# katotetsuro/chainer-maskrcnn

Hardware: AMD Instinct MI355X
Metric: images/sec (1024^2 COCO, bs=2/GPU) at 1/2/4/8 MI355X; ROIAlign bwd HBM GB/s (higher is better)
Workload: dtype f32

## Files before the change

__graft_entry__.py:

```python
import os
import subprocess
import sys

ROOT = os.path.dirname(os.path.abspath(__file__))
PKG = os.path.join(ROOT, 'chainer-maskrcnn_amd')
for _p in (ROOT, PKG):
    if _p not in sys.path:
        sys.path.insert(0, _p)


def build():
    csrc = os.path.join(PKG, 'csrc')
    subprocess.check_call(['make', '-C', csrc, '-j8'])
    oc = os.path.join(ROOT, 'oracle', 'c')
    if os.path.exists(os.path.join(oc, 'Makefile')):
        subprocess.check_call(['make', '-C', oc])
    from chainer_maskrcnn import _hip
    _hip._lib = None
    assert _hip.lib().mrcnn_abi_version() == _hip.ABI_VERSION


def smoke():
    import numpy as np
    import torch
    from chainer_maskrcnn.functions.roi_align_2d_yx import _roi_align_2d_yx
    from oracle import roi_align as ora
    if not torch.cuda.is_available():
        raise RuntimeError('smoke() needs a HIP device')
    rs = np.random.RandomState(0)
    x = rs.standard_normal((1, 256, 25, 34)).astype(np.float32)
    yx = np.array([[0, 10, 20, 300, 400], [0, 0, 0, 399, 543], [0, 100.5, 50.25, 130, 90]], np.float32)
    gy = rs.standard_normal((3, 256, 7, 7)).astype(np.float32)
    xt = torch.from_numpy(x).cuda().contiguous(memory_format=torch.channels_last).requires_grad_(True)
    y = _roi_align_2d_yx(xt, torch.from_numpy(yx).cuda(), 7, 7, 1. / 16)
    y.backward(torch.from_numpy(gy).cuda())
    xy = yx[:, [0, 2, 1, 4, 3]]
    np.testing.assert_array_equal(y.detach().cpu().numpy(), ora.roi_align_fwd(x, xy, 7, 7, 1. / 16, 2))
    np.testing.assert_allclose(xt.grad.cpu().numpy(), ora.roi_align_bwd(gy, xy, x.shape, 1. / 16, 2),
                               rtol=1e-5, atol=1e-4)
    print('smoke ok: roi_align fwd bit-exact, bwd within 1e-5 of the oracle')
    _smoke_train_step()


def _smoke_train_step():
    import numpy as np
    import torch
    from chainer_maskrcnn.model.maskrcnn import MaskRCNN
    from chainer_maskrcnn.model.fpn_maskrcnn_train_chain import FPNMaskRCNNTrainChain, calc_mask_loss
    from chainer_maskrcnn.optimizers import MomentumSGD, WeightDecay
    from chainer_maskrcnn.utils.synthetic import make_batch
    from oracle.model import OracleStep, D
    dev = 'cuda:0'
    stages = (1, 1, 1, 1)
    m = MaskRCNN(n_fg_class=80, device=dev, seed=3, _test_shrink=dict(stages=stages, width_div=2))
    chain = FPNMaskRCNNTrainChain(m, mask_loss_fun=calc_mask_loss, gemm_arithmetic='bf16x6_behind_backbone')
    opt = MomentumSGD(lr=1e-3, momentum=0.9).setup(chain)
    opt.add_hook(WeightDecay(0.0005))
    b = make_batch(3, 2, 128, 160, G=3)
    b['bboxes'][:, :, 2:] = np.minimum(b['bboxes'][:, :, 2:], [128, 160])
    bt = {k: torch.from_numpy(v).to(dev) for k, v in b.items()}
    params = {n: m.ps.p(n).detach().cpu().to(D) for n in m.ps.names()}
    opt.update(chain, bt['imgs'], bt['bboxes'], bt['labels'], bt['masks'], 1.0)
    obs = {k: float(v) for k, v in chain.observation.items()}
    t = {k: v.cpu().numpy() for k, v in chain.targets.items() if torch.is_tensor(v)}
    t['gt_rpn_loc'], t['gt_rpn_label'] = (x.cpu().numpy() for x in chain.rpn_targets)
    t['mask_rois_xy5'], t['mask_levels'], t['mask_label'] = (x.cpu().numpy() for x in chain.mask_inputs)
    img4 = torch.cat([torch.from_numpy(b['imgs']).permute(0, 2, 3, 1), torch.zeros((2, 128, 160, 1))], -1).to(D)
    with torch.no_grad():
        out = OracleStep(params, stages, m.head.n_class, m.head.LOC0).losses(img4, t)
    for k in ('rpn_loc_loss', 'rpn_cls_loss', 'roi_loc_loss', 'roi_cls_loss', 'mask_loss'):
        want = float(out[k])
        assert abs(obs[k] - want) <= 1e-4 * max(abs(want), 1e-3), (k, obs[k], want)
    assert torch.isfinite(m.ps.params).all()
    print('smoke ok: training step losses within 1e-4 of the oracle: %s' % {k: round(v, 5) for k, v in obs.items()})


if __name__ == '__main__':
    build()
    if len(sys.argv) > 1 and sys.argv[1] == 'smoke':
        smoke()
```

chainer-maskrcnn_amd/chainer_maskrcnn/_hip/nn.py:

```python
import torch

from chainer_maskrcnn import _hip
from chainer_maskrcnn._hip import lib, check, ptr, stream_ptr

_ws_cache = {}

PROFILE = None
LOGICAL = None


class _prof(object):
    def __init__(self, kind, n_out_pix, KH, KW, cin, cout, geom=None):
        self.on = PROFILE is not None
        if self.on:
            pass_ = {'fwd': 0, 'bwd_data': 1, 'bwd_filter': 2}[kind]
            executed = lib().mrcnn_conv2d_executed_macs(*geom, pass_) if geom is not None else n_out_pix * KH * KW * cin * cout
            if LOGICAL is not None:
                cin, cout = LOGICAL
            self.rec = [kind, n_out_pix * KH * KW * cin * cout, torch.cuda.Event(enable_timing=True),
                        torch.cuda.Event(enable_timing=True), (n_out_pix, KH, cin, cout), executed, geom,
                        winograd_pass_tiles(),
                        split_operands()]

    def __enter__(self):
# ... 29 lines not shown
        buf = torch.empty(max(int(nbytes), 1 << 20), dtype=torch.uint8, device=device)
        _ws_cache[key] = buf
    return buf


def winograd_pass_tiles():
    import ctypes
    t = (ctypes.c_int * 3)()
    check(lib().mrcnn_conv2d_get_winograd_pass_tiles(t))
    return (t[0], t[1], t[2])


def split_operands():
    import ctypes
    t = (ctypes.c_int * 3)()
    check(lib().mrcnn_conv2d_get_split_operands(t))
    return (t[0], t[1], t[2])


def set_winograd_pass_tiles(fwd, bwd_data, bwd_filter):
    check(lib().mrcnn_conv2d_set_winograd_pass_tiles(int(fwd), int(bwd_data), int(bwd_filter)))


def conv_out(n, k, s, p):
    return (n + 2 * p - k) // s + 1


CONV_PLAN_FIELDS = ('path', 'bm', 'bn', 'ksplit', 'tail_ks', 'wino_m', 'smallc', 'arithmetic', 'plane_gemm')
CONV_PATHS = ('direct', 'split_k', 'tail_split', 'winograd')


def conv_plan(pass_, x_shape, w_shape, stride, pad):
    import ctypes
    N, H, W, Cin = x_shape
    Cout, KH, KW, _ = w_shape
    out = (ctypes.c_int * len(CONV_PLAN_FIELDS))()
    check(lib().mrcnn_conv2d_plan_query(int(pass_), N, H, W, Cin, Cout, KH, KW, stride, pad, out, len(CONV_PLAN_FIELDS)))
    return dict(zip(CONV_PLAN_FIELDS, out))


def conv2d_fwd_raw(x, w, b, stride, pad, relu, keep_v=False):
    _hip.require_cuda(x, w)
    N, H, W, Cin = x.shape
    Cout, KH, KW, Cin2 = w.shape
    assert Cin == Cin2, (x.shape, w.shape)
    assert x.is_contiguous() and w.is_contiguous()
    y = torch.empty((N, conv_out(H, KH, stride, pad), conv_out(W, KW, stride, pad), Cout),
                    dtype=torch.float32, device=x.device)
    nb = lib().mrcnn_conv2d_workspace_bytes(N, H, W, Cin, Cout, KH, KW, stride, pad)
    ws = workspace(nb, x.device) if nb else None
    v = None
    if keep_v:
        vb = lib().mrcnn_conv2d_winograd_v_bytes(N, H, W, Cin, Cout, KH, KW, stride, pad)
        if vb:
            v = torch.empty((vb // 4,), dtype=torch.float32, device=x.device)
    with _prof('fwd', N * y.shape[1] * y.shape[2], KH, KW, Cin, Cout, (N, H, W, Cin, Cout, KH, KW, stride, pad)):
        check(lib().mrcnn_conv2d_fwd_f32(ptr(x), ptr(w), ptr(b), ptr(y), N, H, W, Cin, Cout, KH, KW,
                                         stride, pad, int(relu), ptr(v), ptr(ws), ws.numel() if ws is not None else 0, stream_ptr()))
    return (y, v) if keep_v else y


def conv2d_fwd_bnstats_raw(x, w, stride, pad, keep_v=False):
    N, H, W, Cin = x.shape
    Cout, KH, KW, _ = w.shape
    rows = lib().mrcnn_conv2d_bnstats_rows(N, H, W, Cin, Cout, KH, KW, stride, pad)
    if rows == 0:
        return None
    assert x.is_contiguous() and w.is_contiguous()
    y = torch.empty((N, conv_out(H, KH, stride, pad), conv_out(W, KW, stride, pad), Cout), dtype=torch.float32, device=x.device)
    part = torch.empty((rows, 2, Cout), dtype=torch.float32, device=x.device)
    nb = lib().mrcnn_conv2d_workspace_bytes(N, H, W, Cin, Cout, KH, KW, stride, pad)
    ws = workspace(nb, x.device) if nb else None
    v = None
    if keep_v:
        vb = lib().mrcnn_conv2d_winograd_v_bytes(N, H, W, Cin, Cout, KH, KW, stride, pad)
        if vb:
            v = torch.empty((vb // 4,), dtype=torch.float32, device=x.device)
    with _prof('fwd', N * y.shape[1] * y.shape[2], KH, KW, Cin, Cout, (N, H, W, Cin, Cout, KH, KW, stride, pad)):
        check(lib().mrcnn_conv2d_fwd_bnstats_f32(ptr(x), ptr(w), ptr(y), N, H, W, Cin, Cout, KH, KW, stride, pad, ptr(part), ptr(v),
                                                 ptr(ws), ws.numel() if ws is not None else 0, stream_ptr()))
    return y, v, part


def winograd_w_bytes(x_shape, w_shape, stride, pad):
    N, H, W, Cin = x_shape
    Cout, KH, KW, _ = w_shape
    return lib().mrcnn_conv2d_winograd_w_bytes(N, H, W, Cin, Cout, KH, KW, stride, pad)


def conv2d_bwd_data_raw(gy, w, x_shape, stride, pad, out=None, relu_x=None, emit_w=False, gb=None, gb_accumulate=False):
    N, H, W, Cin = x_shape
    Cout, KH, KW, _ = w.shape
    assert gy.is_contiguous()
    acc = out is not None
    gx = out if acc else torch.empty(x_shape, dtype=torch.float32, device=gy.device)
    nb = lib().mrcnn_conv2d_workspace_bytes(N, H, W, Cin, Cout, KH, KW, stride, pad)
    ws = workspace(nb, gy.device) if nb else None
    wt = None
    if emit_w:
        wb = lib().mrcnn_conv2d_winograd_w_bytes(N, H, W, Cin, Cout, KH, KW, stride, pad)
        assert wb > 0, 'emit_w: the layer does not take the Winograd path'
        wt = torch.empty((wb // 4,), dtype=torch.float32, device=gy.device)
    with _prof('bwd_data', N * gy.shape[1] * gy.shape[2], KH, KW, Cin, Cout, (N, H, W, Cin, Cout, KH, KW, stride, pad)):
        check(lib().mrcnn_conv2d_bwd_data_f32(ptr(gy), ptr(w), ptr(gx), ptr(relu_x), N, H, W, Cin, Cout, KH, KW,
                                              stride, pad, int(acc), ptr(wt), ptr(gb) if emit_w else None, int(gb_accumulate),
                                              ptr(ws), ws.numel() if ws is not None else 0, stream_ptr()))
    return (gx, wt) if emit_w else gx


def conv2d_bwd_filter_raw(x, gy, w_shape, stride, pad, want_bias, gw=None, gb=None, accumulate=None, wino_v=None,
                          wino_w=None):
    N, H, W, Cin = x.shape
    Cout, KH, KW, _ = w_shape
    assert gy.is_contiguous() and x.is_contiguous()
    acc = (gw is not None) if accumulate is None else bool(accumulate)
    if gw is None:
        gw = torch.empty(w_shape, dtype=torch.float32, device=x.device)
        gb = torch.empty((Cout,), dtype=torch.float32, device=x.device) if want_bias else None
    nbytes = lib().mrcnn_conv2d_bwd_filter_workspace_bytes(N, H, W, Cin, Cout, KH, KW, stride, pad)
    ws = workspace(nbytes, x.device)
    with _prof('bwd_filter', N * gy.shape[1] * gy.shape[2], KH, KW, Cin, Cout, (N, H, W, Cin, Cout, KH, KW, stride, pad)):
        check(lib().mrcnn_conv2d_bwd_filter_f32(ptr(x), ptr(gy), ptr(gw), ptr(gb) if want_bias else None, N, H, W, Cin,
                                                Cout, KH, KW, stride, pad, int(acc), ptr(wino_v), ptr(wino_w), ptr(ws), ws.numel(),
                                                stream_ptr()))
    return gw, gb
```

chainer-maskrcnn_amd/chainer_maskrcnn/_hip/ops.py:

```python
import ctypes

import numpy as np
import torch

from chainer_maskrcnn import _hip
from chainer_maskrcnn._hip import lib, check, ptr, stream_ptr
from chainer_maskrcnn._hip.nn import workspace

f32 = torch.float32
i32 = torch.int32


def _empty(shape, dev, dtype=f32):
    return torch.empty(shape, dtype=dtype, device=dev)


def _ck(*ts):
    _hip.require_cuda(*ts)
    for t in ts:
        if t is not None and not t.is_contiguous():
            raise ValueError('non-contiguous tensor passed to a HIP op')


def bn_train_fwd(x, gamma, beta, residual=None, relu=False, running_mean=None, running_var=None,
                 eps=2e-5, decay=0.9):
    _ck(x, gamma, beta, residual)
    C = x.shape[-1]
    P = x.numel() // C
    y = torch.empty_like(x)
    mean = _empty((C,), x.device)
    invstd = _empty((C,), x.device)
    nb = lib().mrcnn_bn_workspace_bytes(P, C)
    ws = workspace(nb, x.device)
    check(lib().mrcnn_bn_train_fwd_f32(ptr(x), ptr(gamma), ptr(beta), ptr(residual), ptr(y), ptr(mean), ptr(invstd),
                                       ptr(running_mean), ptr(running_var), P, C, eps, decay, int(relu), ptr(ws),
                                       ws.numel(), stream_ptr()))
    return y, mean, invstd


def bn_train_fwd_stats(x, part, gamma, beta, residual=None, relu=False, running_mean=None, running_var=None, eps=2e-5, decay=0.9):
    _ck(x, part, gamma, beta, residual)
    C = x.shape[-1]
    P = x.numel() // C
    y = torch.empty_like(x)
    mean = _empty((C,), x.device)
    invstd = _empty((C,), x.device)
    check(lib().mrcnn_bn_train_fwd_stats_f32(ptr(x), ptr(part), part.shape[0], ptr(gamma), ptr(beta), ptr(residual), ptr(y), ptr(mean),
                                             ptr(invstd), ptr(running_mean), ptr(running_var), P, C, eps, decay, int(relu), stream_ptr()))
    return y, mean, invstd


def bn_train_bwd(gy, x, y, gamma, mean, invstd, relu=False, want_gres=False, beta=None, gg=None, gb=None):
    _ck(gy, x, y, gamma, mean, invstd, beta, gg, gb)
    C = x.shape[-1]
    P = x.numel() // C
    gx = torch.empty_like(x)
    gres = torch.empty_like(x) if want_gres else None
    gg = _empty((C,), x.device) if gg is None else gg
    gb = _empty((C,), x.device) if gb is None else gb
    ws = workspace(lib().mrcnn_bn_workspace_bytes(P, C), x.device)
    check(lib().mrcnn_bn_train_bwd_f32(ptr(gy), ptr(x), ptr(y), ptr(gamma), ptr(beta), ptr(mean), ptr(invstd), ptr(gx), ptr(gres),
                                       ptr(gg), ptr(gb), P, C, int(relu), ptr(ws), ws.numel(), stream_ptr()))
    return gx, gres, gg, gb


def bn_infer_fwd(x, gamma, beta, mean, var, residual=None, relu=False, eps=2e-5):
    _ck(x, gamma, beta, mean, var, residual)
    C = x.shape[-1]
    y = torch.empty_like(x)
    check(lib().mrcnn_bn_infer_fwd_f32(ptr(x), ptr(gamma), ptr(beta), ptr(mean), ptr(var), ptr(residual), ptr(y),
                                       x.numel() // C, C, eps, int(relu), stream_ptr()))
    return y


def bn_frozen_bwd(gy, gamma, var, yx=None, beta=None, mean=None, relu=0, want_gres=False, out=None, eps=2e-5):
    _ck(gy, gamma, var, yx, beta, mean, out)
    C = gy.shape[-1]
    gx = torch.empty_like(gy) if out is None else out
    gres = torch.empty_like(gy) if want_gres else None
    check(lib().mrcnn_bn_frozen_bwd_f32(ptr(gy), ptr(yx), ptr(gamma), ptr(beta), ptr(mean), ptr(var), ptr(gx), ptr(gres),
                                        gy.numel() // C, C, eps, int(relu), stream_ptr()))
    return gx, gres


def bn_infer_fwd_pair(xa, gamma_a, beta_a, mean_a, var_a, xb, gamma_b, beta_b, mean_b, var_b, eps=2e-5):
    _ck(xa, gamma_a, beta_a, mean_a, var_a, xb, gamma_b, beta_b, mean_b, var_b)
    if xa.shape != xb.shape:
        raise ValueError('bn_infer_fwd_pair: xa %r and xb %r differ in shape' % (tuple(xa.shape), tuple(xb.shape)))
    C = xa.shape[-1]
    y = torch.empty_like(xa)
    check(lib().mrcnn_bn_infer_fwd_pair_f32(ptr(xa), ptr(gamma_a), ptr(beta_a), ptr(mean_a), ptr(var_a), ptr(xb), ptr(gamma_b),
                                            ptr(beta_b), ptr(mean_b), ptr(var_b), ptr(y), xa.numel() // C, C, eps, stream_ptr()))
    return y


def bn_frozen_bwd_pair(gy, y, gamma_a, var_a, gamma_b, var_b, out_a=None, eps=2e-5):
    _ck(gy, y, gamma_a, var_a, gamma_b, var_b, out_a)
    C = gy.shape[-1]
    gxa = torch.empty_like(gy) if out_a is None else out_a
    gxb = torch.empty_like(gy)
    check(lib().mrcnn_bn_frozen_bwd_pair_f32(ptr(gy), ptr(y), ptr(gamma_a), ptr(var_a), ptr(gamma_b), ptr(var_b), ptr(gxa), ptr(gxb),
                                             gy.numel() // C, C, eps, stream_ptr()))
    return gxa, gxb


GN_PATHS = ('register', 'generic')


def group_norm_plan(R, H, W, C, Cp, G):
    path, nb = ctypes.c_int(-1), ctypes.c_size_t(0)
    check(lib().mrcnn_group_norm_plan(int(R), int(H), int(W), int(C), int(Cp), int(G), ctypes.byref(path), ctypes.byref(nb)))
    return path.value, nb.value


def group_norm_fwd(x, gamma, beta, C, G, relu=False, want_stats=True, eps=1e-5):
    _ck(x, gamma, beta)
    R, H, W, Cp = x.shape
    y = torch.empty_like(x)
    mean = _empty((R, G), x.device) if want_stats else None
    rstd = _empty((R, G), x.device) if want_stats else None
    check(lib().mrcnn_group_norm_fwd_f32(ptr(x), ptr(gamma), ptr(beta), R, H, W, int(C), Cp, int(G), eps, int(bool(relu)), ptr(y),
                                         ptr(mean), ptr(rstd), stream_ptr()))
    return y, mean, rstd


def group_norm_bwd(gy, x, gamma, beta, mean, rstd, C, G, relu=False, gg=None, gb=None, accumulate_params=False):
    _ck(gy, x, gamma, beta, mean, rstd, gg, gb)
    R, H, W, Cp = x.shape
    if tuple(gy.shape) != tuple(x.shape):
        raise ValueError('group_norm_bwd: gy %r and x %r differ in shape' % (tuple(gy.shape), tuple(x.shape)))
    if (gg is None or gb is None) and accumulate_params:
        raise ValueError('group_norm_bwd: accumulate_params needs gg and gb')
    gx = torch.empty_like(x)
    gg = _empty((Cp,), x.device) if gg is None else gg
    gb = _empty((Cp,), x.device) if gb is None else gb
    _, nb = group_norm_plan(R, H, W, C, Cp, G)
    if R == 0 and not accumulate_params:
        gg.zero_()
        gb.zero_()
    ws = workspace(nb, x.device)
    check(lib().mrcnn_group_norm_bwd_f32(ptr(gy), ptr(x), ptr(gamma), ptr(beta), ptr(mean), ptr(rstd), R, H, W, int(C), Cp, int(G),
                                         int(bool(relu)), ptr(gx), ptr(gg), ptr(gb), int(bool(accumulate_params)), ptr(ws), ws.numel(),
                                         stream_ptr()))
    return gx, gg, gb


# ... 857 lines not shown
```

chainer-maskrcnn_amd/chainer_maskrcnn/model/extractor/feature_pyramid_network.py:

```python
from chainer_maskrcnn.nn.core import Conv, BatchNorm, Bottleneck, ParamStore
from chainer_maskrcnn._hip import ops, nn as hnn

MASK_IN_PRODUCER = True
LATERALS_OFF_THE_CHAIN = False
_lat_streams = {}


def _lateral_stream(device):
    import torch
    key = (device.type, device.index)
    if key not in _lat_streams:
        _lat_streams[key] = torch.cuda.Stream(device=device)
    return _lat_streams[key]


class FeaturePyramidNetwork(object):
    feat_strides = [4, 8, 16, 32, 64]
    spatial_scales = list(map(lambda x: 1. / x, feat_strides))
    anchor_base = 16
    anchor_sizes = [32, 64, 128, 256, 512]
    anchor_scales = list(map(lambda x: x / 16., anchor_sizes))

    STAGES = (('res2', 3, 64, 64, 256, 1), ('res3', 4, 256, 128, 512, 2),
              ('res4', 6, 512, 256, 1024, 2), ('res5', 3, 1024, 512, 2048, 2))

    def __init__(self, ps=None, prefix='extractor', stages=None, width_div=1):
        self.ps = ps if ps is not None else ParamStore()
        p = prefix + '/'
        d = width_div
        self.conv1 = Conv(self.ps, p + 'resnet/conv1', 3, 64 // d, 7, 2, 3, bias=True, in_backbone=True)
        self.bn1 = BatchNorm(self.ps, p + 'resnet/bn1', 64 // d)
        self.stages = []
        for si, (name, n, cin, mid, cout, stride) in enumerate(self.STAGES):
            n = n if stages is None else stages[si]
            cin, mid, cout = cin // d, mid // d, cout // d
            blocks = [Bottleneck(self.ps, p + 'resnet/%s/a' % name, cin, mid, cout, stride, True)]
            for i in range(1, n):
                blocks.append(Bottleneck(self.ps, p + 'resnet/%s/b%d' % (name, i), cout, mid, cout, 1, False))
            self.stages.append(blocks)
        fc = 256 // d
        self.out_channels = fc
        self.toplayer = Conv(self.ps, p + 'toplayer', 2048 // d, fc, 1)
        self.conv_p4 = Conv(self.ps, p + 'conv_p4', fc, fc, 3, 1, 1, fwd_tile=0)
        self.conv_p3 = Conv(self.ps, p + 'conv_p3', fc, fc, 3, 1, 1, fwd_tile=0)
        self.conv_p2 = Conv(self.ps, p + 'conv_p2', fc, fc, 3, 1, 1, fwd_tile=0)
        self.conv_p6 = Conv(self.ps, p + 'conv_p6', fc, fc, 1, 2, 0)
        self.lat_p4 = Conv(self.ps, p + 'lat_p4', 1024 // d, fc, 1)
        self.lat_p3 = Conv(self.ps, p + 'lat_p3', 512 // d, fc, 1)
        self.lat_p2 = Conv(self.ps, p + 'lat_p2', 256 // d, fc, 1)
        self.anchor_scales = list(map(lambda x: x / float(self.anchor_base), self.anchor_sizes))
        self.freeze_bn, self.freeze_at = False, 0

    def set_freeze(self, bn=False, at=0):
        at = int(at)
        if not 0 <= at <= 5:
            raise ValueError('freeze_at must be in 0..5 (0 = off, 1 = stem, k = stem + res2 .. res{k}), got %r' % (at,))
        if at > 0 and not bn:
            raise ValueError('freeze_at > 0 requires freeze_bn: a frozen prefix with batch-statistics BatchNorm is not implemented')
        self.freeze_bn, self.freeze_at = bool(bn), at
        self.bn1.frozen = bool(bn)
        names = set()
        for si, blocks in enumerate(self.stages):
            for b in blocks:
                b.trained = si + 2 > at
                for n in b.norms():
                    n.frozen = bool(bn)
        if bn:
            names.update(n for n in self.ps.offsets if '/resnet/' in n and (n.endswith('/gamma') or n.endswith('/beta')))
        for pre in self.frozen_prefixes():
            names.update(n for n in self.ps.offsets if n.startswith(pre + '/'))
        return names

    def frozen_prefixes(self):
        if self.freeze_at < 1:
            return []
        out = [self.conv1.name, self.bn1.name]
        for si in range(min(self.freeze_at - 1, len(self.stages))):
            out += [b.conv1.name.rsplit('/', 1)[0] for b in self.stages[si]]
        return out

    def __call__(self, x):
        t = {}
        stem_trained = self.freeze_at < 1
        h, t['conv1'] = self.conv1.fwd(x, tape=stem_trained)
        h, t['bn1'] = self.bn1.fwd(h, relu=True)
        if stem_trained:
            t['pool_in'] = h
        else:
            t['bn1'] = None
        h = ops.maxpool2x2_fwd(h)
        cs = []
        t['blocks'] = []
        off_chain = LATERALS_OFF_THE_CHAIN and x.is_cuda and hnn.PROFILE is None
        lat = {}
        if off_chain:
            import torch
            main, side = torch.cuda.current_stream(x.device), hnn.side_stream(x.device)
        for si, blocks in enumerate(self.stages):
            for b in blocks:
                h, ctx = b.fwd(h)
                if b.trained:
                    t['blocks'].append((b, ctx))
            cs.append(h)
            if off_chain and si < 3:
                side.wait_stream(main)
                with torch.cuda.stream(side):
                    lat[si] = (self.lat_p2, self.lat_p3, self.lat_p4)[si].fwd(h)
        c2, c3, c4, c5 = cs
        if off_chain:
            main.wait_stream(side)
            for l_, _ in lat.values():
                l_.record_stream(main)
        p5, t['top'] = self.toplayer.fwd(c5)
        l4, t['lat4'] = lat[2] if off_chain else self.lat_p4.fwd(c4)
        m4 = ops.upsample2x_add_fwd(p5, l4)
        p4, t['p4'] = self.conv_p4.fwd(m4)
        l3, t['lat3'] = lat[1] if off_chain else self.lat_p3.fwd(c3)
        m3 = ops.upsample2x_add_fwd(p4, l3)
        p3, t['p3'] = self.conv_p3.fwd(m3)
        l2, t['lat2'] = lat[0] if off_chain else self.lat_p2.fwd(c2)
        m2 = ops.upsample2x_add_fwd(p3, l2)
        p2, t['p2'] = self.conv_p2.fwd(m2)
        p6, t['p6'] = self.conv_p6.fwd(p5)
        self.tape = t
        return p2, p3, p4, p5, p6

    def backward(self, grads, progress=None):
        t = self.tape
        g_p2, g_p3, g_p4, g_p5, g_p6 = grads
        self.conv_p6.bwd(t['p6'], g_p6, gx_acc=g_p5)
        g_m2 = self.conv_p2.bwd(t['p2'], g_p2)
        ops.upsample2x_bwd(g_m2, gtop=g_p3)
        off_chain = LATERALS_OFF_THE_CHAIN and g_p2.is_cuda and hnn.PROFILE is None
        if off_chain:
            import torch
            main, ls = torch.cuda.current_stream(g_p2.device), _lateral_stream(g_p2.device)

        k = self.freeze_at

        def lateral_bwd(conv, ctx, g_m, stage):
            if k >= stage:
                conv.bwd(ctx, g_m, need_gx=False)
                return None
            if not off_chain:
                return conv.bwd(ctx, g_m, mask_gx=MASK_IN_PRODUCER)
            ls.wait_stream(main)
            g_m.record_stream(ls)
            with torch.cuda.stream(ls):
                g_c = conv.bwd(ctx, g_m, mask_gx=MASK_IN_PRODUCER)
            g_c.record_stream(main)
            return g_c
        g_c2 = lateral_bwd(self.lat_p2, t['lat2'], g_m2, 2)
        g_m3 = self.conv_p3.bwd(t['p3'], g_p3)
        ops.upsample2x_bwd(g_m3, gtop=g_p4)
        g_c3 = lateral_bwd(self.lat_p3, t['lat3'], g_m3, 3)
        g_m4 = self.conv_p4.bwd(t['p4'], g_p4)
        ops.upsample2x_bwd(g_m4, gtop=g_p5)
        g_c4 = lateral_bwd(self.lat_p4, t['lat4'], g_m4, 4)
        g_c5 = self.toplayer.bwd(t['top'], g_p5, need_gx=k < 5, mask_gx=MASK_IN_PRODUCER)
        if progress:
            progress(self.toplayer.name)
        acc_for = {id(self.stages[k][0]): g for k, g in ((1, g_c2), (2, g_c3), (3, g_c4))}
        g = g_c5
        first = t['blocks'][0][0] if t['blocks'] else None
        for b, ctx in reversed(t['blocks']):
            if off_chain and acc_for.get(id(b)) is not None:
                main.wait_stream(ls)
            if k >= 1 and b is first:
                g = b.bwd(ctx, g, gy_masked=MASK_IN_PRODUCER, need_gx=False)
            else:
                g = b.bwd(ctx, g, gx_acc=acc_for.get(id(b)), gy_masked=MASK_IN_PRODUCER, mask_gx=MASK_IN_PRODUCER and b is not first)
            if progress:
                progress(b.conv1.name)
        if k >= 1:
            if progress:
                for blocks in reversed(self.stages[:k - 1]):
                    for b in reversed(blocks):
                        progress(b.conv1.name)
            self.tape = None
            return
        g = ops.maxpool2x2_bwd(t['pool_in'], g)
        g, _ = self.bn1.bwd(t['bn1'], g)
        self.conv1.bwd(t['conv1'], g, need_gx=False)
        self.tape = None
```

chainer-maskrcnn_amd/chainer_maskrcnn/nn/core.py:

```python
import math

import numpy as np
import torch

from chainer_maskrcnn._hip import nn as hnn
from chainer_maskrcnn._hip import ops


TRAIN = True

FILTER_GRAD_ON_SIDE_STREAM = True
WINOGRAD_SHARED_GY_TRANSFORM = False
LAYER_TILE_HINTS = True
FWD_TILE_RULE = None
FUSE_BN_STATS = True
FWD_EMULATION_BEHIND_BACKBONE = True
FWD_EMULATION_IN_BACKBONE = True
COMPOSITE_BLOCKS = True


class _layer_tiles(object):
    def __init__(self, conv):
        self.t = FWD_TILE_RULE(conv.name) if FWD_TILE_RULE is not None else (conv.fwd_tile if LAYER_TILE_HINTS else None)
        self.keep = None
# ... 89 lines not shown
    def _view(self, flat, name):
        cache = self._views.get(id(flat))
        if cache is None or cache[0] is not flat:
            self._views = {k: c for k, c in self._views.items() if c[0] is self.params or c[0] is self.grads or c[0] is self.momentum}
            cache = self._views[id(flat)] = (flat, {})
        v = cache[1].get(name)
        if v is None:
            o, shape = self.offsets[name]
            v = cache[1][name] = flat[o:o + int(np.prod(shape))].view(shape)
        return v

    def p(self, name):
        return self._view(self.params, name)

    def g(self, name):
        return self._view(self.grads, name)

    def names(self):
        return list(self.offsets)

    def n_params(self):
        return sum(int(np.prod(s)) for _, s in self.offsets.values())


def lecun_normal(fan_in):
    return lambda shape: (lambda rs: rs.standard_normal(shape) * (1.0 / math.sqrt(fan_in)))


def normal(std):
    return lambda shape: (lambda rs: rs.standard_normal(shape) * std)


class Conv(object):

    def __init__(self, ps, name, cin, cout, k=1, stride=1, pad=0, bias=True, relu=False, init=None,
                 cin_p=None, cout_p=None, cout_index=None, fwd_tile=None, in_backbone=None):
        self.ps, self.name, self.fwd_tile = ps, name, fwd_tile
        self.in_backbone = ('/resnet/' in name) if in_backbone is None else bool(in_backbone)
        self.cin, self.cout, self.k, self.stride, self.pad, self.relu = cin, cout, k, stride, pad, relu
        self.cin_p = cin_p or (4 if cin <= 4 else pad_to(cin, 32))
        self.cout_p = cout_p or pad_to(cout, 32)
        self.has_bias = bias
        idx = np.arange(cout) if cout_index is None else np.asarray(cout_index)
        fan_in = cin * k * k
        gen = (init or lecun_normal(fan_in))((cout, k, k, cin))

        def w_init(rs):
            w = np.zeros((self.cout_p, k, k, self.cin_p), np.float32)
            w[idx, :, :, :cin] = gen(rs)
            return w
        ps.register(name + '/W', (self.cout_p, k, k, self.cin_p), w_init)
        if bias:
            ps.register(name + '/b', (self.cout_p,), lambda rs: np.zeros((self.cout_p,), np.float32))

    @property
    def W(self):
        return self.ps.p(self.name + '/W')

    @property
    def b(self):
        return self.ps.p(self.name + '/b') if self.has_bias else None

    def fwd(self, x, relu=None, bn_stats=False, tape=True):
        relu = self.relu if relu is None else relu
        self.last_bn_part = None
        hnn.LOGICAL = (self.cin, self.cout)
        if not tape:
            with _layer_tiles(self):
                y = hnn.conv2d_fwd_raw(x, self.W, self.b, self.stride, self.pad, relu)
            hnn.LOGICAL = None
            return y, None
        if bn_stats and FUSE_BN_STATS and TRAIN and not relu and not self.has_bias:
            with _layer_tiles(self):
                res = hnn.conv2d_fwd_bnstats_raw(x, self.W, self.stride, self.pad, keep_v=True)
            if res is not None:
                hnn.LOGICAL = None
                y, v, self.last_bn_part = res
                return y, (x, None, v)
        with _layer_tiles(self):
            y, v = hnn.conv2d_fwd_raw(x, self.W, self.b, self.stride, self.pad, relu, keep_v=True) if TRAIN else \
                (hnn.conv2d_fwd_raw(x, self.W, self.b, self.stride, self.pad, relu), None)
        hnn.LOGICAL = None
        return y, (x, y if relu else None, v)

    def bwd(self, ctx, gy, need_gx=True, gx_acc=None, accumulate_params=False, gy_masked=False, mask_gx=False):
        with _layer_tiles(self):
            return self._bwd(ctx, gy, need_gx, gx_acc, accumulate_params, gy_masked, mask_gx)

    def _bwd(self, ctx, gy, need_gx, gx_acc, accumulate_params, gy_masked, mask_gx):
        x, y, v = ctx
        if y is not None and not gy_masked:
            gy = ops.relu_bwd(gy, y)
        gw = self.ps.g(self.name + '/W')
        gb = self.ps.g(self.name + '/b') if self.has_bias else None
        hnn.LOGICAL = (self.cin, self.cout)
        try:
            if WINOGRAD_SHARED_GY_TRANSFORM and need_gx and self.stride == 1 and hnn.winograd_w_bytes(tuple(x.shape), tuple(gw.shape), 1, self.pad) > 0:
                assert not (mask_gx and gx_acc is not None)
                gx, wt = hnn.conv2d_bwd_data_raw(gy, self.W, tuple(x.shape), 1, self.pad, out=gx_acc, relu_x=x if mask_gx else None,
                                                 emit_w=True, gb=gb, gb_accumulate=accumulate_params)
                main = torch.cuda.current_stream(gy.device)
                side = hnn.side_stream(gy.device) if (FILTER_GRAD_ON_SIDE_STREAM and hnn.PROFILE is None) else main
                side.wait_stream(main)
                with torch.cuda.stream(side):
                    hnn.conv2d_bwd_filter_raw(x, gy, tuple(gw.shape), 1, self.pad, False, gw=gw, gb=None,
                                              accumulate=accumulate_params, wino_v=v, wino_w=wt)
                if side is not main:
                    for t_ in (gy, x, v, wt):
                        if t_ is not None:
                            t_.record_stream(side)
                return gx
            if FILTER_GRAD_ON_SIDE_STREAM and hnn.PROFILE is None:
                main = torch.cuda.current_stream(gy.device)
                side = hnn.side_stream(gy.device)
                side.wait_stream(main)
                with torch.cuda.stream(side):
                    hnn.conv2d_bwd_filter_raw(x, gy, tuple(gw.shape), self.stride, self.pad, self.has_bias, gw=gw, gb=gb,
                                              accumulate=accumulate_params, wino_v=v)
                gy.record_stream(side)
                x.record_stream(side)
                if v is not None:
                    v.record_stream(side)
            else:
                hnn.conv2d_bwd_filter_raw(x, gy, tuple(gw.shape), self.stride, self.pad, self.has_bias, gw=gw, gb=gb,
                                          accumulate=accumulate_params, wino_v=v)
            if not need_gx:
                return None
            if self.stride == 1:
                assert not (mask_gx and gx_acc is not None) or self.k == 1
                return hnn.conv2d_bwd_data_raw(gy, self.W, tuple(x.shape), 1, self.pad, out=gx_acc,
                                               relu_x=x if mask_gx else None)
            assert self.k == 1 and self.pad == 0, 'strided backward-data only for 1x1 convolutions'
            g_sub = self.bwd_data_sub(gy)
        finally:
            hnn.LOGICAL = None
        return ops.subsample_bwd(g_sub, tuple(x.shape), self.stride, gx=gx_acc, relu_x=x if mask_gx else None)

    def bwd_data_sub(self, gy, out=None):
        N, Ho, Wo, _ = gy.shape
        keep = hnn.LOGICAL
        hnn.LOGICAL = (self.cin, self.cout)
        g = hnn.conv2d_bwd_data_raw(gy, self.W, (N, Ho, Wo, self.cin_p), 1, 0, out=out)
        hnn.LOGICAL = keep
        return g


class BatchNorm(object):

    def __init__(self, ps, name, c):
        self.ps, self.name, self.c = ps, name, c
        self.frozen = False
        ps.register(name + '/gamma', (c,), lambda rs: np.ones((c,), np.float32))
        ps.register(name + '/beta', (c,), lambda rs: np.zeros((c,), np.float32))
        ps.register(name + '/avg_mean', (c,), lambda rs: np.zeros((c,), np.float32), trainable=False)
        ps.register(name + '/avg_var', (c,), lambda rs: np.ones((c,), np.float32), trainable=False)

    def fwd(self, x, relu=False, residual=None, partials=None):
        gamma, beta = self.ps.p(self.name + '/gamma'), self.ps.p(self.name + '/beta')
        if not TRAIN or self.frozen:
            y = ops.bn_infer_fwd(x, gamma, beta, self.ps.buffers[self.name + '/avg_mean'], self.ps.buffers[self.name + '/avg_var'],
                                 residual, relu)
            if not TRAIN:
                return y, None
            return y, ('frozen', y if relu else None)
        if partials is not None and partials.shape[2] == x.shape[-1]:
            y, mean, invstd = ops.bn_train_fwd_stats(x, partials, gamma, beta, residual, relu, self.ps.buffers[self.name + '/avg_mean'],
                                                     self.ps.buffers[self.name + '/avg_var'])
        else:
            y, mean, invstd = ops.bn_train_fwd(x, gamma, beta, residual, relu, self.ps.buffers[self.name + '/avg_mean'],
                                               self.ps.buffers[self.name + '/avg_var'])
        return y, (x, y if (residual is not None or not relu) else None, mean, invstd, relu)

    def scale_operands(self):
        return self.ps.p(self.name + '/gamma'), self.ps.buffers[self.name + '/avg_var']

    def bwd(self, ctx, gy, want_gres=False, gy_masked=False, in_place=False):
        if ctx[0] == 'frozen':
            y = None if gy_masked else ctx[1]
            assert not (want_gres and y is None)
            gamma, var = self.scale_operands()
            return ops.bn_frozen_bwd(gy, gamma, var, yx=y, relu=0 if y is None else 1, want_gres=want_gres, out=gy if in_place else None)
        x, y, mean, invstd, relu = ctx
        if gy_masked:
            assert relu and not want_gres
            relu, y = False, None
        gx, gres, _, _ = ops.bn_train_bwd(gy, x, y, self.ps.p(self.name + '/gamma'), mean, invstd, relu, want_gres,
                                          beta=self.ps.p(self.name + '/beta'), gg=self.ps.g(self.name + '/gamma'),
                                          gb=self.ps.g(self.name + '/beta'))
        return gx, gres


class GroupNorm(object):

    def __init__(self, ps, name, c, groups=32):
        if groups < 1 or c % groups != 0:
            raise ValueError('GroupNorm %s: %d groups do not divide %d channels' % (name, groups, c))
        self.ps, self.name, self.c, self.groups = ps, name, c, groups
        self.c_p = pad_to(c, 32)

        def ones(rs):
            g = np.zeros((self.c_p,), np.float32)
            g[:c] = 1.0
            return g
        ps.register(name + '/gamma', (self.c_p,), ones)
        ps.register(name + '/beta', (self.c_p,), lambda rs: np.zeros((self.c_p,), np.float32))

    def fwd(self, x, relu=False):
        gamma, beta = self.ps.p(self.name + '/gamma'), self.ps.p(self.name + '/beta')
        y, mean, rstd = ops.group_norm_fwd(x, gamma, beta, self.c, self.groups, relu=relu, want_stats=TRAIN)
        return y, ((x, mean, rstd, relu) if TRAIN else None)

    def bwd(self, ctx, gy, gy_masked=False, accumulate_params=False):
        x, mean, rstd, relu = ctx
        gx, _, _ = ops.group_norm_bwd(gy, x, self.ps.p(self.name + '/gamma'), self.ps.p(self.name + '/beta'), mean, rstd, self.c,
                                      self.groups, relu=bool(relu) and not gy_masked, gg=self.ps.g(self.name + '/gamma'),
                                      gb=self.ps.g(self.name + '/beta'), accumulate_params=accumulate_params)
        return gx


class Bottleneck(object):

    def __init__(self, ps, name, cin, mid, cout, stride, project):
        self.project, self.stride = project, stride
        he = lambda fan_in: (lambda shape: (lambda rs: rs.standard_normal(shape) * math.sqrt(2.0 / fan_in)))
        self.conv1 = Conv(ps, name + '/conv1', cin, mid, 1, stride, 0, bias=False, init=he(cin), in_backbone=True)
        self.bn1 = BatchNorm(ps, name + '/bn1', mid)
        self.conv2 = Conv(ps, name + '/conv2', mid, mid, 3, 1, 1, bias=False, init=he(mid * 9), in_backbone=True)
        self.bn2 = BatchNorm(ps, name + '/bn2', mid)
        self.conv3 = Conv(ps, name + '/conv3', mid, cout, 1, 1, 0, bias=False, init=he(mid), in_backbone=True)
        self.bn3 = BatchNorm(ps, name + '/bn3', cout)
        if project:
            self.conv4 = Conv(ps, name + '/conv4', cin, cout, 1, stride, 0, bias=False, init=he(cin), in_backbone=True)
            self.bn4 = BatchNorm(ps, name + '/bn4', cout)
        self.trained = True

    def norms(self):
        return [self.bn1, self.bn2, self.bn3] + ([self.bn4] if self.project else [])

    def _fwd_frozen(self, x):
        t = self.trained
        h1, c1 = self.conv1.fwd(x, tape=t)
        a1, b1 = self.bn1.fwd(h1, relu=True)
        h2, c2 = self.conv2.fwd(a1, tape=t)
        a2, b2 = self.bn2.fwd(h2, relu=True)
        h3, c3 = self.conv3.fwd(a2, tape=t)
        if self.project:
            h4, c4 = self.conv4.fwd(x, tape=t)
            ps, n3, n4 = self.bn3.ps, self.bn3.name, self.bn4.name
            y = ops.bn_infer_fwd_pair(h3, ps.p(n3 + '/gamma'), ps.p(n3 + '/beta'), ps.buffers[n3 + '/avg_mean'], ps.buffers[n3 + '/avg_var'],
                                      h4, ps.p(n4 + '/gamma'), ps.p(n4 + '/beta'), ps.buffers[n4 + '/avg_mean'], ps.buffers[n4 + '/avg_var'])
            b3 = ('frozen', y)
        else:
            c4 = None
            y, b3 = self.bn3.fwd(h3, relu=True, residual=x)
        if not t:
# ... 161 lines not shown
```

chainer-maskrcnn_amd/csrc/conv.hip:

```cpp
#include "common.h"
#include "bn_common.h"
#include <algorithm>
#include <cstdlib>

namespace {

typedef float f32x16 __attribute__((ext_vector_type(16)));

constexpr int BK = 32;
constexpr int LDK = BK + 4;
constexpr int CONV_THREADS = 256;

enum { MODE_FWD = 0, MODE_BWD_DATA = 1, MODE_BWD_FILTER = 2 };

struct ConvP {
    const float *a;
    const float *b;
    float *c;
    const float *bias;
    const float *relu_x;
    int N, H, W, Cin;
    int Ho, Wo, Cout;
    int KH, KW, stride, pad;
    int pad_w;
// ... 1178 lines not shown
    if (M_ == 2) {
        r[0] = D[0] + 0.5f * (D[1] + D[2]); r[1] = 0.5f * (D[1] - D[2]); r[2] = 0.5f * (D[1] + D[2]) + D[3];
    } else {
        const float p12 = D[1] + D[2], m12 = D[1] - D[2], p34 = D[3] + D[4], m34 = D[3] - D[4];
        r[0] = (0.25f * D[0] - p12 * (1.0f / 6.0f)) + p34 * (1.0f / 24.0f);
        r[1] = m34 * (1.0f / 12.0f) - m12 * (1.0f / 6.0f);
        r[2] = (p34 * (1.0f / 6.0f) - p12 * (1.0f / 6.0f)) + D[5];
    }
}

template <int M_>
__device__ __forceinline__ void wino_filter_body(const float *__restrict__ w, float *__restrict__ U, int Cout, int Cin,
                                                 int transposed, unsigned blk, int uplanes = 0) {
    constexpr int A_ = M_ + 2;
    const int i = (int)(blk * 256u + threadIdx.x);
    if (i >= Cout * Cin) return;
    const int ci = transposed ? i / Cout : i % Cin, co = transposed ? i % Cout : i / Cin;
    float t[A_][3];
#pragma unroll
    for (int v = 0; v < 3; ++v) {
        float g[3], c[A_];
#pragma unroll
        for (int u = 0; u < 3; ++u) {
            const int uu = transposed ? 2 - u : u, vv = transposed ? 2 - v : v;
            g[u] = w[(((size_t)co * 3 + uu) * 3 + vv) * Cin + ci];
        }
        wino_g<M_>(g, c);
#pragma unroll
        for (int r = 0; r < A_; ++r) t[r][v] = c[r];
    }
    const size_t stride = (size_t)Cout * Cin;
    const size_t o = transposed ? (size_t)ci * Cout + co : (size_t)co * Cin + ci;
    if (uplanes) {
        const unsigned rows = transposed ? (unsigned)Cin : (unsigned)Cout, cols = transposed ? (unsigned)Cout : (unsigned)Cin;
        const unsigned rr = transposed ? (unsigned)ci : (unsigned)co, cc = transposed ? (unsigned)co : (unsigned)ci;
        unsigned short *Up = reinterpret_cast<unsigned short *>(U);
#pragma unroll
        for (int r = 0; r < A_; ++r) {
            float row[A_];
            wino_g<M_>(t[r], row);
#pragma unroll
            for (int q = 0; q < A_; ++q) {
                const unsigned off = pg_off_r4((unsigned)(r * A_ + q) * rows + rr, cc & ~3u, cols) / 2u + (cc & 3u);
                const float v = row[q];
                const __bf16 h = (__bf16)v;
                const float r1 = v - (float)h;
                const __bf16 m = (__bf16)r1;
                const __bf16 l = (__bf16)(r1 - (float)m);
                Up[off] = __builtin_bit_cast(unsigned short, h);
                Up[off + 64] = __builtin_bit_cast(unsigned short, m);
                Up[off + 128] = __builtin_bit_cast(unsigned short, l);
            }
        }
        return;
    }
#pragma unroll
    for (int r = 0; r < A_; ++r) {
        float row[A_];
        wino_g<M_>(t[r], row);
#pragma unroll
        for (int q = 0; q < A_; ++q) U[(size_t)(r * A_ + q) * stride + o] = row[q];
    }
}
template <int M_>
__global__ __launch_bounds__(256) void k_wino_filter(const float *__restrict__ w, float *__restrict__ U, int Cout, int Cin,
                                                     int transposed, int uplanes) {
    wino_filter_body<M_>(w, U, Cout, Cin, transposed, blockIdx.x, uplanes);
}

typedef unsigned u32x4 __attribute__((ext_vector_type(4)));
__device__ __forceinline__ V4 v4buf(__amdgpu_buffer_rsrc_t rs, unsigned voff, unsigned soff) {
    const u32x4 v = __builtin_amdgcn_raw_buffer_load_b128(rs, voff, soff, 0);
    return {__uint_as_float(v.x), __uint_as_float(v.y), __uint_as_float(v.z), __uint_as_float(v.w)};
}
__device__ __forceinline__ V4 v4buf_nt(__amdgpu_buffer_rsrc_t rs, unsigned voff, unsigned soff) {
    const u32x4 v = __builtin_amdgcn_raw_buffer_load_b128(rs, voff, soff, 2);
    return {__uint_as_float(v.x), __uint_as_float(v.y), __uint_as_float(v.z), __uint_as_float(v.w)};
}
__device__ __forceinline__ void v4bufst(__amdgpu_buffer_rsrc_t rs, unsigned voff, unsigned soff, V4 v) {
    const u32x4 d = {__float_as_uint(v.x), __float_as_uint(v.y), __float_as_uint(v.z), __float_as_uint(v.w)};
    __builtin_amdgcn_raw_buffer_store_b128(d, rs, voff, soff, 0);
}
struct InBN { const float *gamma, *beta, *mean, *invstd; };
template <int M_>
__device__ __forceinline__ void wino_input_body(const float *__restrict__ x, float *__restrict__ V, int N, int H, int W, int C,
                                                int th, int tw, long long T, long long Tp, unsigned blk, const InBN bn = InBN{},
                                                int panel = 0) {
    constexpr int A_ = M_ + 2;
    const unsigned C4 = (unsigned)C / 4u;
    const unsigned i = blk * 256u + threadIdx.x;
    if (i >= (unsigned)Tp * C4) return;
    unsigned t = i / C4;
    const int c = (int)(i - t * C4) * 4;
    const unsigned ks = (unsigned)((size_t)Tp * C * 4);
    const auto rsV = __builtin_amdgcn_make_buffer_rsrc((void *)V, 0, (unsigned)((size_t)A_ * A_ * Tp * C * 4), 0x00020000);
    if (panel > 1 && t < (unsigned)T) {
        const unsigned per = (unsigned)th * (unsigned)tw, pw = (unsigned)panel;
        const unsigned n0 = t / per, q = t - n0 * per;
        const unsigned full = (unsigned)tw / pw * pw, nf = (unsigned)th * full;
        unsigned ty0, tx0;
        if (q < nf) {
            const unsigned pp = q / ((unsigned)th * pw), r = q - pp * (unsigned)th * pw;
            ty0 = r / pw; tx0 = pp * pw + (r - ty0 * pw);
        } else {
            const unsigned wr = (unsigned)tw - full, q2 = q - nf;
            ty0 = q2 / wr; tx0 = full + (q2 - ty0 * wr);
        }
        t = n0 * per + ty0 * (unsigned)tw + tx0;
    }
    const unsigned vo = (unsigned)(((size_t)t * C + c) * 4);
    if (t >= (unsigned)T) {
#pragma unroll
        for (int k = 0; k < A_ * A_; ++k) v4bufst(rsV, vo + (unsigned)k * ks, 0, v4zero());
        return;
    }
    const unsigned trow = t / (unsigned)tw;
    const int tx = (int)(t - trow * (unsigned)tw);
    const int n = (int)(trow / (unsigned)th);
    const int ty = (int)(trow - (unsigned)n * (unsigned)th);
    const auto rsX = __builtin_amdgcn_make_buffer_rsrc((void *)x, 0, (unsigned)((size_t)N * H * W * C * 4), 0x00020000);
    const unsigned OOB = 0xFFFFFFFFu;
    unsigned rowo[A_], colo[A_];
#pragma unroll
    for (int r = 0; r < A_; ++r) {
        const int h = M_ * ty - 1 + r, ww = M_ * tx - 1 + r;
        rowo[r] = (unsigned)h < (unsigned)H ? (unsigned)(((size_t)n * H + h) * W * C * 4) : OOB;
        colo[r] = (unsigned)ww < (unsigned)W ? (unsigned)(((size_t)ww * C + c) * 4) : OOB;
    }
    V4 bg = v4zero(), bb = v4zero(), bm = v4zero(), bs = v4zero();
    if (bn.gamma) { bg = v4ld(bn.gamma + c); bb = v4ld(bn.beta + c); bm = v4ld(bn.mean + c); bs = v4ld(bn.invstd + c); }
    V4 b[A_][A_];
#pragma unroll
    for (int q = 0; q < A_; ++q) {
        V4 d[A_], r[A_];
#pragma unroll
        for (int rr = 0; rr < A_; ++rr) d[rr] = v4buf(rsX, (rowo[rr] == OOB || colo[q] == OOB) ? OOB : rowo[rr] + colo[q], 0);
        if (bn.gamma) {
#pragma unroll
            for (int rr = 0; rr < A_; ++rr) {
                const bool in = !(rowo[rr] == OOB || colo[q] == OOB);
                const V4 v = d[rr];
                V4 o;
                o.x = relu1(bn_affine1(v.x, bg.x, bm.x, bs.x, bb.x)); o.y = relu1(bn_affine1(v.y, bg.y, bm.y, bs.y, bb.y));
                o.z = relu1(bn_affine1(v.z, bg.z, bm.z, bs.z, bb.z)); o.w = relu1(bn_affine1(v.w, bg.w, bm.w, bs.w, bb.w));
                d[rr] = in ? o : v4zero();
            }
        }
        wino_bt<M_, V4>(d, r);
#pragma unroll
        for (int rr = 0; rr < A_; ++rr) b[rr][q] = r[rr];
    }
#pragma unroll
    for (int rr = 0; rr < A_; ++rr) {
        V4 row[A_];
        wino_bt<M_, V4>(b[rr], row);
#pragma unroll
        for (int q = 0; q < A_; ++q) v4bufst(rsV, vo + (unsigned)(rr * A_ + q) * ks, 0, row[q]);
    }
}
__device__ __forceinline__ unsigned xcd_banded(unsigned g, unsigned first, unsigned nb, int on) {
    const unsigned b = g - first;
    if (!on) return b;
    const unsigned f0 = first & 7u, n2 = nb + f0, b2 = b + f0;
    const unsigned q = n2 >> 3, r = n2 & 7u, xcd = b2 & 7u;
    const unsigned v2 = (xcd < r ? xcd * (q + 1) : r * (q + 1) + (xcd - r) * q) + (b2 >> 3);
    return v2 - min(xcd + 1u, f0);
}
template <int M_>
__global__ __launch_bounds__(256) void k_wino_input(const float *__restrict__ x, float *__restrict__ V, int N, int H, int W, int C,
                                                    int th, int tw, long long T, long long Tp, int banded, InBN bn) {
    wino_input_body<M_>(x, V, N, H, W, C, th, tw, T, Tp, xcd_banded(blockIdx.x, 0, gridDim.x, banded), bn, banded);
}
template <int M_>
__global__ __launch_bounds__(256) void k_wino_input_filter(const float *__restrict__ x, float *__restrict__ V, int N, int H, int W, int C,
                                                           int th, int tw, long long T, long long Tp, const float *__restrict__ w,
                                                           float *__restrict__ U, int Cout_w, int Cin_w, int transposed, unsigned fblocks,
                                                           int banded, int uplanes, InBN bn) {
    if (blockIdx.x < fblocks) wino_filter_body<M_>(w, U, Cout_w, Cin_w, transposed, blockIdx.x, uplanes);
    else wino_input_body<M_>(x, V, N, H, W, C, th, tw, T, Tp, xcd_banded(blockIdx.x, fblocks, gridDim.x - fblocks, banded), bn, banded);
}

template <int M_>
__global__ __launch_bounds__(256) void k_wino_output(const float *__restrict__ Mb, float *__restrict__ y, int N, int H, int W, int C,
                                                     int th, int tw, long long T, long long Tp, const float *__restrict__ bias,
                                                     int relu, int accumulate, const float *__restrict__ relu_x,
                                                     float *__restrict__ bn_part) {
    constexpr int A_ = M_ + 2;
    __shared__ float4 sred[2][256];
    const unsigned C4 = (unsigned)C / 4u;
    const unsigned i = blockIdx.x * 256u + threadIdx.x;
    V4 bs = v4zero(), bq = v4zero();
    if (i < (unsigned)T * C4) {
        const unsigned t = i / C4;
        const int c = (int)(i - t * C4) * 4;
        const unsigned trow = t / (unsigned)tw;
        const int tx = (int)(t - trow * (unsigned)tw);
        const int n = (int)(trow / (unsigned)th);
        const int ty = (int)(trow - (unsigned)n * (unsigned)th);
        const unsigned ks = (unsigned)((size_t)Tp * C * 4);
        const auto rsM = __builtin_amdgcn_make_buffer_rsrc((void *)Mb, 0, (unsigned)((size_t)A_ * A_ * Tp * C * 4), 0x00020000);
        const unsigned ybytes = (unsigned)((size_t)N * H * W * C * 4);
        const auto rsY = __builtin_amdgcn_make_buffer_rsrc((void *)y, 0, ybytes, 0x00020000);
        const auto rsR = __builtin_amdgcn_make_buffer_rsrc((void *)relu_x, 0, relu_x ? ybytes : 0u, 0x00020000);
        const unsigned mo = (unsigned)(((size_t)t * C + c) * 4);
        V4 s[M_][A_];
#pragma unroll
        for (int q = 0; q < A_; ++q) {
            V4 m[A_], r[M_];
#pragma unroll
            for (int rr = 0; rr < A_; ++rr) m[rr] = v4buf_nt(rsM, mo, (unsigned)(rr * A_ + q) * ks);
            wino_at<M_, V4>(m, r);
#pragma unroll
            for (int a = 0; a < M_; ++a) s[a][q] = r[a];
        }
        const V4 bv = bias ? v4ld(bias + c) : v4zero();
        const unsigned OOB = 0xFFFFFFFFu;
#pragma unroll
        for (int a = 0; a < M_; ++a) {
            V4 row[M_], old[M_], xm[M_];
            wino_at<M_, V4>(s[a], row);
            const int h = M_ * ty + a;
            unsigned off[M_];
#pragma unroll
            for (int b = 0; b < M_; ++b) {
                const int ww = M_ * tx + b;
                off[b] = (h < H && ww < W) ? (unsigned)((((size_t)n * H + h) * W + ww) * C + c) * 4u : OOB;
            }
            if (accumulate) {
#pragma unroll
                for (int b = 0; b < M_; ++b) old[b] = v4buf(rsY, off[b], 0);
            }
            if (relu_x) {
#pragma unroll
                for (int b = 0; b < M_; ++b) xm[b] = v4buf(rsR, off[b], 0);
            }
#pragma unroll
            for (int b = 0; b < M_; ++b) {
                V4 v = row[b] + bv;
                if (relu) { v.x = fmaxf(v.x, 0.f); v.y = fmaxf(v.y, 0.f); v.z = fmaxf(v.z, 0.f); v.w = fmaxf(v.w, 0.f); }
                if (accumulate) v = v + old[b];
                if (relu_x) {
                    v.x = xm[b].x > 0.f ? v.x : 0.f; v.y = xm[b].y > 0.f ? v.y : 0.f; v.z = xm[b].z > 0.f ? v.z : 0.f; v.w = xm[b].w > 0.f ? v.w : 0.f;
                }
                v4bufst(rsY, off[b], 0, v);
                if (off[b] != OOB) {
                    bs = bs + v;
                    bq.x = fmaf(v.x, v.x, bq.x); bq.y = fmaf(v.y, v.y, bq.y); bq.z = fmaf(v.z, v.z, bq.z); bq.w = fmaf(v.w, v.w, bq.w);
                }
            }
        }
    }
    if (bn_part) {
        sred[0][threadIdx.x] = make_float4(bs.x, bs.y, bs.z, bs.w);
        sred[1][threadIdx.x] = make_float4(bq.x, bq.y, bq.z, bq.w);
        __syncthreads();
        if (threadIdx.x < C4) {
            float4 a = sred[0][threadIdx.x], b2 = sred[1][threadIdx.x];
            for (unsigned k = threadIdx.x + C4; k < 256; k += C4) {
                const float4 q = sred[0][k], r = sred[1][k];
                a.x += q.x; a.y += q.y; a.z += q.z; a.w += q.w;
                b2.x += r.x; b2.y += r.y; b2.z += r.z; b2.w += r.w;
            }
// ... 172 lines not shown
#pragma unroll
        for (int j = 0; j < A_; ++j) Dall[q][j] = dU[o0 + (size_t)(q * A_ + j) * Cin];
    for (int sl = 1; sl < nslab; ++sl) {
        const float *ds = dU + (size_t)sl * Cout * (A_ * A_) * Cin + o0;
#pragma unroll
        for (int q = 0; q < A_; ++q)
#pragma unroll
            for (int j = 0; j < A_; ++j) Dall[q][j] += ds[(size_t)(q * A_ + j) * Cin];
    }
    float old[3][3];
    if (accumulate) {
#pragma unroll
        for (int u = 0; u < 3; ++u)
#pragma unroll
            for (int v = 0; v < 3; ++v) old[u][v] = gw[(((size_t)co * 3 + u) * 3 + v) * Cin + ci];
    }
    float r[3][A_];
#pragma unroll
    for (int j = 0; j < A_; ++j) {
        float D[A_], c3[3];
#pragma unroll
        for (int q = 0; q < A_; ++q) D[q] = Dall[q][j];
        wino_gt<M_>(D, c3);
#pragma unroll
        for (int u = 0; u < 3; ++u) r[u][j] = c3[u];
    }
#pragma unroll
    for (int u = 0; u < 3; ++u) {
        float o[3];
        wino_gt<M_>(r[u], o);
#pragma unroll
        for (int v = 0; v < 3; ++v) gw[(((size_t)co * 3 + u) * 3 + v) * Cin + ci] = accumulate ? old[u][v] + o[v] : o[v];
    }
}

#define WINO_LAUNCH(KERN, G, GRID, ...)                                                              \
    do {                                                                                             \
        if (g_debug_skip & 2) break;                                                                 \
        if ((G).m == 2) hipLaunchKernelGGL((KERN<2>), GRID, dim3(256), 0, st, __VA_ARGS__);          \
        else hipLaunchKernelGGL((KERN<4>), GRID, dim3(256), 0, st, __VA_ARGS__);                     \
        MRCNN_LAUNCH_CHECK();                                                                        \
    } while (0)

#define WINO_LAUNCH_OUT(G, GRID, ...) WINO_LAUNCH(k_wino_output, G, GRID, __VA_ARGS__)

int g_pg_big = 1, g_pg_min_tiles = 256;
bool pg_big_g_ok(const WinoGeom &g, int Cin, int Cout) {
    if (g_split_mode[PASS_BWD_FILTER] != 3 || !g_pg_big) return false;
    if (Cout % PGB_BM || Cin % PGB_BN || g.Tp % 32) return false;
    return g.Tp >= 2048 && (long long)g.nk * g.Tp * Cout * 6 < (1ll << 32) && (long long)g.nk * g.Tp * Cin * 4 < (1ll << 32);
}
struct WinoFLayout { size_t v, w, slabs, du, total; WinoGeom g; int ksplit, kchunk; int big; int ks32, kc32; };
ConvP wino_filter_p(const WinoGeom &g, int Cin, int Cout) {
    ConvP p = make_p(1, 1, (int)g.Tp, Cin, Cout, 1, 1, 1, 0);
    p.wbatch_rows = (int)g.Tp; p.wbatch_n = g.nk;
    bwd_filter_gemm(p);
    return p;
}
WinoFLayout wino_filter_layout(int N, int H, int W, int Cin, int Cout) {
    WinoFLayout L;
    L.g = wino_geom(N, H, W, PASS_BWD_FILTER);
    ConvP p = wino_filter_p(L.g, Cin, Cout);
    filter_plan(p, L.ksplit, L.kchunk);
    L.ks32 = L.ksplit; L.kc32 = L.kchunk;
    L.big = pg_big_g_ok(L.g, Cin, Cout) ? 1 : 0;
    if (L.big) {
        const long long tiles = (long long)L.g.nk * (Cout / PGB_BM) * (Cin / PGB_BN);
        long long ks = std::max(1ll, (long long)g_cus() / tiles);
        ks = std::min(ks, std::max(1ll, L.g.Tp / 256));
        L.kchunk = (int)((L.g.Tp / 32 + ks - 1) / ks * 32);
        L.ksplit = (int)((L.g.Tp + L.kchunk - 1) / L.kchunk);
    }
    auto al = [](size_t b) { return (b + 255) / 256 * 256; };
    size_t o = 0;
    L.v = o; o += al((size_t)L.g.nk * L.g.Tp * Cin * 4);
    L.w = o; o += al((size_t)L.g.nk * L.g.Tp * Cout * 6);
    L.slabs = o; o += al((size_t)std::max(L.ksplit, L.ks32) * Cout * L.g.nk * Cin * 4);
    L.du = o; o += al((size_t)Cout * L.g.nk * Cin * 4);
    L.total = o;
    return L;
}

thread_local InBN t_inbn{};

int wino_bwd_filter(const float *x, const float *gy, float *gw, int N, int H, int W, int Cin, int Cout, int accumulate, void *ws,
                    hipStream_t st, const float *v_cached, const float *w_cached, float *bias_part = nullptr, int *bias_rows = nullptr) {
    const InBN inbn = t_inbn;
    const WinoFLayout L = wino_filter_layout(N, H, W, Cin, Cout);
    const WinoGeom &g = L.g;
    char *base = (char *)ws;
    float *Vw = (float *)(base + L.v), *Wt = (float *)(base + L.w), *slabs = (float *)(base + L.slabs), *dU = (float *)(base + L.du);
    const float *V = v_cached ? v_cached : Vw;
    const long long nin = g.Tp * (Cin / 4), nout = g.Tp * (Cout / 4);
    if (!v_cached) WINO_LAUNCH(k_wino_input, g, dim3((unsigned)((nin + 255) / 256)), x, Vw, N, H, W, Cin, g.th, g.tw, g.T, g.Tp, g_wino_banded, inbn);
    const int C4o = Cout / 4;
    const bool fuse_bias = bias_part && bias_rows && !w_cached && C4o <= 256 && 256 % C4o == 0 && !(g_debug_skip & 2);
    if (bias_rows) *bias_rows = fuse_bias ? (int)((nout + 255) / 256) : 0;
    const int big = (L.big && !w_cached) ? 1 : 0;
    if (!w_cached) WINO_LAUNCH(k_wino_gy, g, dim3((unsigned)((nout + 255) / 256)), gy, Wt, N, H, W, Cout, g.th, g.tw, g.T, g.Tp,
                               fuse_bias ? bias_part : (float *)nullptr, big);
    if (big) {
        PlaneGemmP q{};
        q.a = reinterpret_cast<const unsigned short *>(Wt); q.b = reinterpret_cast<const unsigned short *>(V);
        q.c = L.ksplit > 1 ? slabs : dU;
        q.M = Cout; q.N = Cin; q.K = (int)g.Tp; q.batch_rows = (int)g.Tp; q.nbatch = g.nk; q.ksplit = L.ksplit; q.kchunk = L.kchunk;
        q.bytes_a = (unsigned)((size_t)g.nk * g.Tp * Cout * 6); q.bytes_b = (unsigned)((size_t)g.nk * g.Tp * Cin * 4);
        q.ldc = g.nk * Cin; q.dbg = 0; q.stamps = nullptr;
        if (!(g_debug_skip & 1)) launch_pgemm<5>(q, PGB_BM, PGB_BN, st);
        MRCNN_LAUNCH_CHECK();
        if (L.ksplit > 1) {
            const size_t n4 = (size_t)Cout * g.nk * Cin / 4;
            if (!(g_debug_skip & 10)) hipLaunchKernelGGL(k_sum_slabs, dim3(mrcnn::cdiv(n4, 256)), dim3(256), 0, st, slabs, dU, n4, L.ksplit, 0);
            MRCNN_LAUNCH_CHECK();
        }
        WINO_LAUNCH(k_wino_filter_grad, g, dim3(mrcnn::cdiv(Cout * Cin, 256)), dU, gw, Cout, Cin, accumulate, 1);
        return 0;
    }
    ConvP p = wino_filter_p(g, Cin, Cout);
    p.ksplit = L.ks32; p.kchunk = L.kc32;
    p.a = w_cached ? w_cached : Wt; p.b = V; p.c = p.ksplit > 1 ? slabs : dU;
    p.bytes_a = (unsigned)((size_t)g.nk * g.Tp * Cout * 4); p.bytes_b = (unsigned)((size_t)g.nk * g.Tp * Cin * 4);
    launch_conv<MODE_BWD_FILTER>(p, g.nk * p.ksplit, filter_tile(p), st);
    MRCNN_LAUNCH_CHECK();
    if (p.ksplit > 1) {
        const size_t n4 = (size_t)Cout * g.nk * Cin / 4;
        if (!(g_debug_skip & 10)) hipLaunchKernelGGL(k_sum_slabs, dim3(mrcnn::cdiv(n4, 256)), dim3(256), 0, st, slabs, dU, n4, p.ksplit, 0);
        MRCNN_LAUNCH_CHECK();
    }
    WINO_LAUNCH(k_wino_filter_grad, g, dim3(mrcnn::cdiv(Cout * Cin, 256)), dU, gw, Cout, Cin, accumulate, 1);
    return 0;
}

bool pg_big_ok(int pass, const WinoGeom &g, int K, int Nn) {
    if (g_split_mode[pass] != 3 || !g_pg_big) return false;
    if (g.Tp % PGB_BM || Nn % PGB_BN || K % 16) return false;
    const long long tiles = (long long)g.nk * g.Tp / PGB_BM * (Nn / PGB_BN);
    const long long rounds = (tiles + g_cus() - 1) / g_cus();
    if (tiles * 10 < rounds * g_cus() * 8) return false;
    return tiles >= g_pg_min_tiles && (long long)g.nk * g.Tp * K * 4 < (1ll << 32) && (long long)g.nk * Nn * K * 6 < (1ll << 32);
}

int wino_gemm_p(ConvP &p, const WinoGeom &g, int Cin, int Cout) {
    p = make_p(1, 1, (int)(g.nk * g.Tp), Cin, Cout, 1, 1, 1, 0);
    p.M = (int)(g.nk * g.Tp); p.Ng = Cout;
    p.wbatch_rows = (int)g.Tp; p.wbatch_n = g.nk;
    return Cin / BK;
}

int wino_conv(const float *in, const float *w, float *out, int N, int H, int W, int Cin, int Cout, bool transposed,
              const float *bias, int relu, int accumulate, const float *relu_x, void *ws, size_t ws_bytes, hipStream_t st,
              float *v_keep, float *w_keep = nullptr, float *gbias = nullptr, int gbias_accumulate = 0, float *bn_part = nullptr) {
    const InBN inbn = transposed ? InBN{} : t_inbn;
    const WinoLayout L = wino_layout(N, H, W, Cin, Cout, transposed ? PASS_BWD_DATA : PASS_FWD);
    const WinoGeom &g = L.g;
    char *base = (char *)ws;
    float *U = (float *)(base + L.u), *V = v_keep ? v_keep : (float *)(base + L.v), *Mb = (float *)(base + L.m);
    const long long nin = g.Tp * (Cin / 4), nout = g.T * (Cout / 4);
    const unsigned fblocks = (unsigned)mrcnn::cdiv(Cout * Cin, 256);
    const int big = pg_big_ok(transposed ? PASS_BWD_DATA : PASS_FWD, g, Cin, Cout) ? 1 : 0;
    if (w_keep) WINO_LAUNCH(k_wino_filter, g, dim3(fblocks), w, U, transposed ? Cin : Cout, transposed ? Cout : Cin, transposed ? 1 : 0, big);
    if (w_keep) {
        const bool wb = gbias && (256 % (Cin / 4)) == 0;
        const int nblk = (int)std::min<long long>((nin + 255) / 256, 512);
        float *bias_part = wb ? (float *)(base + L.m) : nullptr;
        WINO_LAUNCH(k_wino_gy_dual, g, dim3(nblk), in, V, w_keep, bias_part, N, H, W, Cin, g.th, g.tw, g.T, g.Tp);
        if (wb) {
            if (!(g_debug_skip & 2)) hipLaunchKernelGGL(k_colsum_final, dim3(mrcnn::cdiv(Cin, CSF_CH)), dim3(CSF_CH * CSF_SL), 0, st, bias_part, gbias, nblk, Cin, gbias_accumulate);
            MRCNN_LAUNCH_CHECK();
        } else if (gbias) {
            const int P = N * H * W;
            const ColPlan cp = col_plan(P, Cin);
            float *part = (float *)(base + L.m);
            if (!(g_debug_skip & 2)) hipLaunchKernelGGL(k_colsum_partial, dim3(cp.nblk), dim3(256), 0, st, in, part, P, Cin, cp.G, cp.RPI, cp.rows_per_blk);
            MRCNN_LAUNCH_CHECK();
            if (!(g_debug_skip & 2)) hipLaunchKernelGGL(k_colsum_final, dim3(mrcnn::cdiv(Cin, CSF_CH)), dim3(CSF_CH * CSF_SL), 0, st, part, gbias, cp.nblk, Cin, gbias_accumulate);
            MRCNN_LAUNCH_CHECK();
        }
    } else
        WINO_LAUNCH(k_wino_input_filter, g, dim3(fblocks + (unsigned)((nin + 255) / 256)), in, V, N, H, W, Cin, g.th, g.tw, g.T, g.Tp, w, U,
                    transposed ? Cin : Cout, transposed ? Cout : Cin, transposed ? 1 : 0, fblocks, g_wino_banded, big, inbn);
    if (big) {
        PlaneGemmP q{};
        q.a = reinterpret_cast<const unsigned short *>(V); q.b = reinterpret_cast<const unsigned short *>(U); q.c = Mb;
        q.M = (int)(g.nk * g.Tp); q.N = Cout; q.K = Cin; q.batch_rows = (int)g.Tp; q.nbatch = g.nk; q.ksplit = 1; q.kchunk = Cin;
        q.bytes_a = (unsigned)((size_t)g.nk * g.Tp * Cin * 4); q.bytes_b = (unsigned)((size_t)g.nk * Cout * Cin * 6);
        q.ldc = Cout; q.dbg = 0; q.stamps = nullptr;
        if (!(g_debug_skip & 1)) launch_pgemm<4>(q, PGB_BM, PGB_BN, st);
        MRCNN_LAUNCH_CHECK();
        WINO_LAUNCH_OUT(g, dim3((unsigned)((nout + 255) / 256)), Mb, out, N, H, W, Cout, g.th, g.tw, g.T, g.Tp, bias, relu,
                    accumulate, relu_x, bn_part);
        return 0;
    }
    ConvP p;
    const int nsteps = wino_gemm_p(p, g, Cin, Cout);
    p.a = V; p.b = U; p.c = Mb;
    p.bytes_a = (unsigned)((size_t)g.nk * g.Tp * Cin * 4); p.bytes_b = (unsigned)((size_t)g.nk * Cout * Cin * 4);
    if (int e = run_data_conv<MODE_FWD>(p, nsteps, Cout, base + L.inner, ws_bytes - L.inner, st)) return e;
    WINO_LAUNCH_OUT(g, dim3((unsigned)((nout + 255) / 256)), Mb, out, N, H, W, Cout, g.th, g.tw, g.T, g.Tp, bias, relu,
                accumulate, relu_x, bn_part);
    return 0;
}

bool fwd_takes_wino(int N, int H, int W, int Cin, int Cout, int KH, int KW, int stride, int pad, bool have_ws, size_t ws_bytes) {
    return wino_ok(N, H, W, Cin, Cout, KH, KW, stride, pad, PASS_FWD) && have_ws && ws_bytes >= wino_ws_bytes(N, H, W, Cin, Cout, PASS_FWD);
}
bool bwd_data_takes_wino(int N, int H, int W, int Cin, int Cout, int KH, int KW, int stride, int pad, bool have_ws, size_t ws_bytes) {
    return wino_ok(N, H, W, Cout, Cin, KH, KW, stride, pad, PASS_BWD_DATA) && have_ws && ws_bytes >= wino_ws_bytes(N, H, W, Cout, Cin, PASS_BWD_DATA);
}
int check_bwd_data(int Cin, int stride) {
    if (stride != 1)
        return mrcnn::fail_arg(MRCNN_E_UNSUPPORTED, "conv2d_bwd_data: stride %d (only 1; strided 1x1 convs are "
                                                    "handled by the host as a subsample + stride-1 conv)", stride);
    if (Cin == 4) return mrcnn::fail_arg(MRCNN_E_UNSUPPORTED, "conv2d_bwd_data: Cin == 4 (image layer) has no data gradient");
    return 0;
}

}

extern "C" size_t mrcnn_conv2d_workspace_bytes(int N, int H, int W, int Cin, int Cout, int KH, int KW, int stride, int pad) {
    if (N <= 0 || H <= 0 || W <= 0 || Cin <= 0 || Cout <= 0 || KH <= 0 || KW <= 0 || stride <= 0 || pad < 0) return 0;
    const long long Ho = conv_out(H, KH, stride, pad), Wo = conv_out(W, KW, stride, pad);
    if (Ho <= 0 || Wo <= 0) return 0;
    const long long a = (long long)N * Ho * Wo * Cout, b = (long long)N * H * W * Cin;
    const long long fill = (long long)g_plan_fill * g_cus();
    const long long cap = fill * 8192;
    long long need = 0;
    if (a < cap) need = std::max(need, a);
    if (b < cap) need = std::max(need, b);
    const size_t tail = (size_t)4 * g_cus() * 128 * 128 * sizeof(float);
    size_t bytes = std::max((size_t)need * 16 * sizeof(float), tail);
    if (wino_ok(N, H, W, Cin, Cout, KH, KW, stride, pad, PASS_FWD)) bytes = std::max(bytes, wino_ws_bytes(N, H, W, Cin, Cout, PASS_FWD));
    if (wino_ok(N, H, W, Cout, Cin, KH, KW, stride, pad, PASS_BWD_DATA)) bytes = std::max(bytes, wino_ws_bytes(N, H, W, Cout, Cin, PASS_BWD_DATA));
    return bytes;
}

extern "C" int mrcnn_debug_conv_parts(int mask) {
    g_dbg_parts = mask & 0xff;
    g_pg_big = (mask & 0x100) ? 0 : 1;
    return 0;
}

extern "C" int mrcnn_debug_split_planes_f32(const float *x, void *planes, int R, int C, int r4, void *stream) {
    if (!x || !planes || R <= 0 || C <= 0 || C % 16 || (long long)R * C * 6 >= (1ll << 32) || (r4 == 1 && R % 4))
        return mrcnn::fail_arg(MRCNN_E_INVALID, "debug_split_planes: null pointer, C %% 16 != 0, R %% 4 != 0 (P16R4) or more than 4 GiB of planes");
    hipLaunchKernelGGL(k_split_planes, dim3(mrcnn::cdiv((long long)R * (C / 4), 256)), dim3(256), 0, (hipStream_t)stream, x,
                       (unsigned short *)planes, (unsigned)R, (unsigned)C, r4);
    MRCNN_LAUNCH_CHECK();
    return 0;
}
static unsigned long long *g_pg_stamps = nullptr;
extern "C" int mrcnn_debug_planes_gemm_stamps(unsigned long long *stamps) {
    g_pg_stamps = stamps;
    return 0;
}
extern "C" int mrcnn_debug_planes_gemm(int kind, const void *a, const void *b, float *c, int M, int N, int K, int batch_rows, int nbatch,
                                       int ksplit, int bm, int bn, void *stream) {
    if (!a || !b || !c || M <= 0 || N <= 0 || K <= 0 || nbatch <= 0 || ksplit <= 0 || kind < 0 || kind > 5)
        return mrcnn::fail_arg(MRCNN_E_INVALID, "debug_planes_gemm: bad arguments");
    PlaneGemmP p{};
    p.a = (const unsigned short *)a; p.b = (const unsigned short *)b; p.c = c;
    p.M = M; p.N = N; p.K = K; p.batch_rows = batch_rows; p.nbatch = nbatch; p.ksplit = ksplit;
// ... 172 lines not shown
                                    int W, int Cin, int Cout, int KH, int KW, int stride, int pad, int relu,
                                    float *wino_v, void *ws, size_t ws_bytes, void *stream) {
    g_cur_pass = 0;
    if (int e = check_conv(x, w, y, N, H, W, Cin, Cout, KH, KW, stride, pad)) return e;
    if (fwd_takes_wino(N, H, W, Cin, Cout, KH, KW, stride, pad, ws != nullptr, ws_bytes))
        return wino_conv(x, w, y, N, H, W, Cin, Cout, false, bias, relu, 0, nullptr, ws, ws_bytes, (hipStream_t)stream, wino_v);
    ConvP p = make_p(N, H, W, Cin, Cout, KH, KW, stride, pad);
    p.a = x; p.b = w; p.c = y; p.bias = bias; p.relu = relu;
    p.bytes_a = (unsigned)((size_t)N * H * W * Cin * 4); p.bytes_b = (unsigned)((size_t)Cout * KH * KW * Cin * 4);
    const int nsteps = fwd_gemm(p);
    return run_data_conv<MODE_FWD>(p, nsteps, Cout, ws, ws_bytes, (hipStream_t)stream);
}

static int bnstats_plan(ConvP &p, TileChoice &t, bool &wino, int N, int H, int W, int Cin, int Cout, int KH, int KW, int stride, int pad) {
    wino = false;
    if (N <= 0 || H <= 0 || W <= 0 || Cin <= 0 || Cout <= 0 || KH <= 0 || KW <= 0 || stride <= 0 || pad < 0) return 0;
    if ((Cin % BK && Cin != 4) || Cout % BK || Cin == 4) return 0;
    if (wino_ok(N, H, W, Cin, Cout, KH, KW, stride, pad, PASS_FWD)) {
        const int C4 = Cout / 4;
        if (C4 > 256 || 256 % C4) return 0;
        wino = true;
        const WinoGeom g = wino_geom(N, H, W, PASS_FWD);
        return (int)((g.T * C4 + 255) / 256);
    }
    p = make_p(N, H, W, Cin, Cout, KH, KW, stride, pad);
    if (p.Ho <= 0 || p.Wo <= 0) return 0;
    p.M = N * p.Ho * p.Wo; p.Ng = Cout;
    data_plan<MODE_FWD>(p, t, KH * KW * (Cin / BK));
    if (p.ksplit > 1 || p.tail_ks) return 0;
    return mrcnn::cdiv(p.M, t.bm) * 2;
}
extern "C" size_t mrcnn_conv2d_bnstats_rows(int N, int H, int W, int Cin, int Cout, int KH, int KW, int stride, int pad) {
    ConvP p;
    TileChoice t;
    bool wino;
    return (size_t)bnstats_plan(p, t, wino, N, H, W, Cin, Cout, KH, KW, stride, pad);
}
extern "C" int mrcnn_conv2d_fwd_bnstats_f32(const float *x, const float *w, float *y, int N, int H, int W, int Cin, int Cout, int KH,
                                            int KW, int stride, int pad, float *bn_part, float *wino_v, void *ws, size_t ws_bytes,
                                            void *stream) {
    g_cur_pass = 0;
    if (int e = check_conv(x, w, y, N, H, W, Cin, Cout, KH, KW, stride, pad)) return e;
    ConvP p;
    TileChoice t;
    bool wino;
    if (!bn_part || bnstats_plan(p, t, wino, N, H, W, Cin, Cout, KH, KW, stride, pad) == 0)
        return mrcnn::fail_arg(MRCNN_E_UNSUPPORTED, "conv2d_fwd_bnstats: no fused statistics for this geometry (mrcnn_conv2d_bnstats_rows == 0)");
    if (wino) {
        if (!ws || ws_bytes < wino_ws_bytes(N, H, W, Cin, Cout, PASS_FWD))
            return mrcnn::fail_arg(MRCNN_E_WORKSPACE, "conv2d_fwd_bnstats: workspace %zu < %zu", ws_bytes, wino_ws_bytes(N, H, W, Cin, Cout, PASS_FWD));
        return wino_conv(x, w, y, N, H, W, Cin, Cout, false, nullptr, 0, 0, nullptr, ws, ws_bytes, (hipStream_t)stream, wino_v, nullptr, nullptr, 0, bn_part);
    }
    p.a = x; p.b = w; p.c = y; p.bias = nullptr; p.relu = 0; p.bn_part = bn_part;
    p.bytes_a = (unsigned)((size_t)N * H * W * Cin * 4); p.bytes_b = (unsigned)((size_t)Cout * KH * KW * Cin * 4);
    launch_conv<MODE_FWD>(p, 1, t, (hipStream_t)stream);
    MRCNN_LAUNCH_CHECK();
    return 0;
}

extern "C" int mrcnn_conv2d_inbn_ok(int N, int H, int W, int Cin, int Cout, int KH, int KW, int stride, int pad) {
    if (N <= 0 || H <= 0 || W <= 0 || Cin <= 0 || Cout <= 0 || KH != 3 || KW != 3 || stride != 1 || pad != 1 || (Cin % 4)) return 0;
    return (wino_ok(N, H, W, Cin, Cout, KH, KW, stride, pad, PASS_FWD) && wino_ok(N, H, W, Cin, Cout, KH, KW, stride, pad, PASS_BWD_FILTER)) ? 1 : 0;
}
static int inbn_args(const float *g, const float *b, const float *m, const float *s, int N, int H, int W, int Cin, int Cout, int KH, int KW, int stride,
                     int pad, const char *who) {
    if (!g || !b || !m || !s) return mrcnn::fail_arg(MRCNN_E_INVALID, "%s: null BatchNorm pointer", who);
    if (!mrcnn_conv2d_inbn_ok(N, H, W, Cin, Cout, KH, KW, stride, pad))
        return mrcnn::fail_arg(MRCNN_E_UNSUPPORTED, "%s: this geometry does not take the Winograd path in both passes (mrcnn_conv2d_inbn_ok == 0)", who);
    return 0;
}
extern "C" int mrcnn_conv2d_fwd_inbn_f32(const float *x, const float *in_gamma, const float *in_beta, const float *in_mean, const float *in_invstd,
                                         const float *w, float *y, int N, int H, int W, int Cin, int Cout, int KH, int KW, int stride, int pad,
                                         float *bn_part, float *wino_v, void *ws, size_t ws_bytes, void *stream) {
    if (int e = inbn_args(in_gamma, in_beta, in_mean, in_invstd, N, H, W, Cin, Cout, KH, KW, stride, pad, "conv2d_fwd_inbn")) return e;
    if (!ws || ws_bytes < wino_ws_bytes(N, H, W, Cin, Cout, PASS_FWD))
        return mrcnn::fail_arg(MRCNN_E_WORKSPACE, "conv2d_fwd_inbn: workspace %zu < %zu", ws_bytes, wino_ws_bytes(N, H, W, Cin, Cout, PASS_FWD));
    t_inbn = InBN{in_gamma, in_beta, in_mean, in_invstd};
    const int rc = bn_part ? mrcnn_conv2d_fwd_bnstats_f32(x, w, y, N, H, W, Cin, Cout, KH, KW, stride, pad, bn_part, wino_v, ws, ws_bytes, stream)
                           : mrcnn_conv2d_fwd_f32(x, w, nullptr, y, N, H, W, Cin, Cout, KH, KW, stride, pad, 0, wino_v, ws, ws_bytes, stream);
    t_inbn = InBN{};
    return rc;
}

extern "C" int mrcnn_conv2d_fwd_rect_f32(const float *x, const float *w, const float *bias, float *y, int N, int H, int W,
                                         int Cin, int Cout, int KH, int KW, int stride, int pad_h, int pad_w, int relu, void *ws,
                                         size_t ws_bytes, void *stream) {
    g_cur_pass = 0;
    if (pad_h < 0 || pad_w < 0) return mrcnn::fail_arg(MRCNN_E_INVALID, "conv2d_fwd_rect: negative padding");
    if (int e = check_conv(x, w, y, N, H, W, Cin, Cout, KH, KW, stride, std::max(pad_h, pad_w))) return e;
    if (conv_out(H, KH, stride, pad_h) <= 0 || conv_out(W, KW, stride, pad_w) <= 0 || Cin == 4)
        return mrcnn::fail_arg(MRCNN_E_INVALID, "conv2d_fwd_rect: empty output (or the 4-channel image layer)");
    ConvP p = make_p(N, H, W, Cin, Cout, KH, KW, stride, pad_h);
    p.pad_w = pad_w;
    p.Wo = conv_out(W, KW, stride, pad_w);
    p.a = x; p.b = w; p.c = y; p.bias = bias; p.relu = relu;
    p.bytes_a = (unsigned)((size_t)N * H * W * Cin * 4); p.bytes_b = (unsigned)((size_t)Cout * KH * KW * Cin * 4);
    p.M = N * p.Ho * p.Wo; p.Ng = Cout;
    return run_data_conv<MODE_FWD>(p, KH * KW * (Cin / BK), Cout, ws, ws_bytes, (hipStream_t)stream);
}

extern "C" size_t mrcnn_conv2d_winograd_w_bytes(int N, int H, int W, int Cin, int Cout, int KH, int KW, int stride, int pad) {
    if (N <= 0 || H <= 0 || W <= 0 || Cin <= 0 || Cout <= 0 || KH <= 0 || KW <= 0 || stride <= 0 || pad < 0) return 0;
    if (!wino_ok(N, H, W, Cout, Cin, KH, KW, stride, pad, PASS_BWD_DATA) || !wino_ok(N, H, W, Cin, Cout, KH, KW, stride, pad, PASS_BWD_FILTER)) return 0;
    const WinoGeom g = wino_geom(N, H, W, PASS_BWD_DATA);
    if (g.m != wino_geom(N, H, W, PASS_BWD_FILTER).m) return 0;
    return (size_t)g.nk * g.Tp * Cout * sizeof(float);
}

extern "C" int mrcnn_conv2d_bwd_data_f32(const float *gy, const float *w, float *gx, const float *relu_x, int N, int H, int W,
                                         int Cin, int Cout, int KH, int KW, int stride, int pad,
                                         int accumulate, float *wino_w, float *gbias, int gbias_accumulate, void *ws,
                                         size_t ws_bytes, void *stream) {
    g_cur_pass = 1;
    if (int e = check_conv(gy, w, gx, N, H, W, Cin, Cout, KH, KW, stride, pad)) return e;
    if (int e = check_bwd_data(Cin, stride)) return e;
    ConvP p = make_p(N, H, W, Cin, Cout, KH, KW, stride, pad);
    if (bwd_data_takes_wino(N, H, W, Cin, Cout, KH, KW, stride, pad, ws != nullptr, ws_bytes))
        return wino_conv(gy, w, gx, N, H, W, Cout, Cin, true, nullptr, 0, accumulate, relu_x, ws, ws_bytes, (hipStream_t)stream, nullptr,
                         wino_w, wino_w ? gbias : nullptr, gbias_accumulate);
    if (wino_w || gbias) return mrcnn::fail_arg(MRCNN_E_UNSUPPORTED, "conv2d_bwd_data: wino_w / gbias only on the Winograd path (mrcnn_conv2d_winograd_w_bytes() > 0)");
    p.a = gy; p.b = w; p.c = gx; p.accumulate = accumulate; p.relu_x = relu_x;
    p.bytes_a = (unsigned)((size_t)N * p.Ho * p.Wo * Cout * 4); p.bytes_b = (unsigned)((size_t)Cout * KH * KW * Cin * 4);
    const int nsteps = bwd_data_gemm(p);
    return run_data_conv<MODE_BWD_DATA>(p, nsteps, Cin, ws, ws_bytes, (hipStream_t)stream);
}

extern "C" size_t mrcnn_conv2d_bwd_filter_workspace_bytes(int N, int H, int W, int Cin, int Cout, int KH, int KW,
                                                          int stride, int pad) {
    if (N <= 0 || H <= 0 || W <= 0 || Cin <= 0 || Cout <= 0 || KH <= 0 || KW <= 0 || stride <= 0 || pad < 0) return 0;
    ConvP p = make_p(N, H, W, Cin, Cout, KH, KW, stride, pad);
    if (p.Ho <= 0 || p.Wo <= 0) return 0;
    int ksplit, kchunk;
    filter_plan(p, ksplit, kchunk);
    const size_t wsz = (size_t)Cout * KH * KW * Cin * sizeof(float);
    const size_t P = (size_t)N * p.Ho * p.Wo;
    const size_t bias_part = (size_t)col_plan((int)P, Cout).nblk * Cout * sizeof(float);
    if (wino_ok(N, H, W, Cin, Cout, KH, KW, stride, pad, PASS_BWD_FILTER)) {
        const WinoFLayout L = wino_filter_layout(N, H, W, Cin, Cout);
        const size_t rows = (size_t)((L.g.Tp * (Cout / 4) + 255) / 256);
        return L.total + std::max(bias_part, rows * Cout * sizeof(float)) + 256;
    }
    return wsz * ksplit + bias_part + 256;
}

extern "C" int mrcnn_conv2d_bwd_filter_f32(const float *x, const float *gy, float *gw, float *gbias, int N,
                                           int H, int W, int Cin, int Cout, int KH, int KW, int stride, int pad,
                                           int accumulate, const float *wino_v, const float *wino_w, void *ws, size_t ws_bytes,
                                           void *stream) {
    g_cur_pass = 2;
    if (int e = check_conv(x, gy, gw, N, H, W, Cin, Cout, KH, KW, stride, pad)) return e;
    if (g_debug_skip & 4) return 0;
    const size_t need = mrcnn_conv2d_bwd_filter_workspace_bytes(N, H, W, Cin, Cout, KH, KW, stride, pad);
    if (!ws || ws_bytes < need) return mrcnn::fail_arg(MRCNN_E_WORKSPACE, "conv2d_bwd_filter: workspace %zu < %zu", ws_bytes, need);
    hipStream_t st = (hipStream_t)stream;
    ConvP p = make_p(N, H, W, Cin, Cout, KH, KW, stride, pad);
    if (wino_ok(N, H, W, Cin, Cout, KH, KW, stride, pad, PASS_BWD_FILTER)) {
        const WinoFLayout L = wino_filter_layout(N, H, W, Cin, Cout);
        if (wino_v && !(wino_ok(N, H, W, Cin, Cout, KH, KW, stride, pad, PASS_FWD) && wino_geom(N, H, W, PASS_FWD).m == L.g.m)) wino_v = nullptr;
        if (wino_w && mrcnn_conv2d_winograd_w_bytes(N, H, W, Cin, Cout, KH, KW, stride, pad) == 0) wino_w = nullptr;
        float *bias_part = (float *)((char *)ws + L.total);
        int bias_rows = 0;
        if (int e = wino_bwd_filter(x, gy, gw, N, H, W, Cin, Cout, accumulate, ws, st, wino_v, wino_w, gbias ? bias_part : nullptr, &bias_rows)) return e;
        if (gbias) {
            int nrows = bias_rows;
            if (nrows == 0) {
                const int P = N * p.Ho * p.Wo;
// ... 47 lines not shown
```

chainer-maskrcnn_amd/csrc/nn.hip:

```cpp
#include "common.h"
#include "bn_common.h"
#include "resize_common.h"

namespace {

constexpr int NT = 256;

struct Nhwc4 { int n, h, w, c; };
__device__ __forceinline__ Nhwc4 split_nhwc4(size_t i, int C4, int Wd, int Hd, bool wide) {
    Nhwc4 r;
    if (!wide) {
        const unsigned u = (unsigned)i, q = u / (unsigned)C4, q2 = q / (unsigned)Wd, q3 = q2 / (unsigned)Hd;
        r.c = (int)(u - q * (unsigned)C4); r.w = (int)(q - q2 * (unsigned)Wd); r.h = (int)(q2 - q3 * (unsigned)Hd); r.n = (int)q3;
    } else {
        const size_t q = i / C4, q2 = q / Wd, q3 = q2 / Hd;
        r.c = (int)(i - q * C4); r.w = (int)(q - q2 * Wd); r.h = (int)(q2 - q3 * Hd); r.n = (int)q3;
    }
    return r;
}

inline int ew_grid(size_t n4) { return (int)std::min<size_t>((n4 + NT - 1) / NT, 256 * 16); }

int g_red_cap = 1024;
struct RedPlan {
// ... 395 lines not shown
        {
            const float4 ga = ld4(gamma_b + c), m = ld4(mean_b + c), s = ld4(invstd_b + c), gb = ld4(gbeta_b + c), gg = ld4(ggamma_b + c);
            st4(gxb + i * 4, bn_bwd_dx4(g, vb, ga, m, s, gb, gg, invP));
        }
    }
}

__global__ __launch_bounds__(NT) void k_relu_bwd(const float *__restrict__ gy, const float *__restrict__ y,
                                                 float *__restrict__ gx, size_t n4) {
    for (size_t i = (size_t)blockIdx.x * NT + threadIdx.x; i < n4; i += (size_t)gridDim.x * NT) {
        st4(gx + i * 4, relu_mask4(ld4(gy + i * 4), ld4(y + i * 4)));
    }
}

__global__ __launch_bounds__(NT) void k_add(const float *__restrict__ a, const float *__restrict__ b,
                                            float *__restrict__ o, size_t n4) {
    for (size_t i = (size_t)blockIdx.x * NT + threadIdx.x; i < n4; i += (size_t)gridDim.x * NT) {
        st4(o + i * 4, add4(ld4(a + i * 4), ld4(b + i * 4)));
    }
}

__global__ __launch_bounds__(NT) void k_maxpool_fwd(const float *__restrict__ x, float *__restrict__ y, int N, int H,
                                                    int W, int C4, int Ho, int Wo) {
    const size_t n4 = (size_t)N * Ho * Wo * C4;
    for (size_t i = (size_t)blockIdx.x * NT + threadIdx.x; i < n4; i += (size_t)gridDim.x * NT) {
        const Nhwc4 ix = split_nhwc4(i, C4, Wo, Ho, n4 > 0xFFFFFFFFull);
        const int c = ix.c, wo = ix.w, ho = ix.h, n = ix.n;
        float4 m = f4(-INFINITY);
#pragma unroll
        for (int dy = 0; dy < 2; ++dy)
#pragma unroll
            for (int dx = 0; dx < 2; ++dx) {
                const int h = 2 * ho + dy, w = 2 * wo + dx;
                if (h < H && w < W) {
                    const float4 v = ld4(x + ((((size_t)n * H + h) * W + w) * C4 + c) * 4);
                    m.x = fmaxf(m.x, v.x); m.y = fmaxf(m.y, v.y); m.z = fmaxf(m.z, v.z); m.w = fmaxf(m.w, v.w);
                }
            }
        st4(y + i * 4, m);
    }
}

__global__ __launch_bounds__(NT) void k_maxpool3s2_fwd(const float *__restrict__ x, float *__restrict__ y, int N, int H, int W,
                                                       int C4, int Ho, int Wo) {
    const size_t n4 = (size_t)N * Ho * Wo * C4;
    for (size_t i = (size_t)blockIdx.x * NT + threadIdx.x; i < n4; i += (size_t)gridDim.x * NT) {
        const Nhwc4 ix = split_nhwc4(i, C4, Wo, Ho, n4 > 0xFFFFFFFFull);
        const int c = ix.c, wo = ix.w, ho = ix.h, n = ix.n;
        float4 m = f4(-INFINITY);
#pragma unroll
        for (int dy = 0; dy < 3; ++dy)
#pragma unroll
            for (int dx = 0; dx < 3; ++dx) {
                const int h = 2 * ho + dy, w = 2 * wo + dx;
                if (h < H && w < W) {
                    const float4 v = ld4(x + ((((size_t)n * H + h) * W + w) * C4 + c) * 4);
                    m.x = fmaxf(m.x, v.x); m.y = fmaxf(m.y, v.y); m.z = fmaxf(m.z, v.z); m.w = fmaxf(m.w, v.w);
                }
            }
        st4(y + i * 4, m);
    }
}

__global__ __launch_bounds__(NT) void k_global_avg_pool(const float *__restrict__ x, float *__restrict__ y, int R, int P, int C4) {
    const size_t n4 = (size_t)R * C4;
    for (size_t i = (size_t)blockIdx.x * NT + threadIdx.x; i < n4; i += (size_t)gridDim.x * NT) {
        const int c = (int)(i % C4), r = (int)(i / C4);
        float4 a = f4(0.f);
        for (int p = 0; p < P; ++p) {
            const float4 v = ld4(x + (((size_t)r * P + p) * C4 + c) * 4);
            a.x += v.x; a.y += v.y; a.z += v.z; a.w += v.w;
        }
        const float d = (float)P;
        st4(y + i * 4, make_float4(a.x / d, a.y / d, a.z / d, a.w / d));
    }
}

__global__ __launch_bounds__(NT) void k_relu_fwd(const float *__restrict__ x, float *__restrict__ y, size_t n4) {
    for (size_t i = (size_t)blockIdx.x * NT + threadIdx.x; i < n4; i += (size_t)gridDim.x * NT) {
        st4(y + i * 4, relu4(ld4(x + i * 4)));
    }
}

__global__ __launch_bounds__(NT) void k_maxpool_bwd(const float *__restrict__ x, const float *__restrict__ gy,
                                                    float *__restrict__ gx, int N, int H, int W, int C4, int Ho, int Wo) {
    const size_t n4 = (size_t)N * Ho * Wo * C4;
    for (size_t i = (size_t)blockIdx.x * NT + threadIdx.x; i < n4; i += (size_t)gridDim.x * NT) {
        const Nhwc4 ix = split_nhwc4(i, C4, Wo, Ho, n4 > 0xFFFFFFFFull);
        const int c = ix.c, wo = ix.w, ho = ix.h, n = ix.n;
        const float4 g = ld4(gy + i * 4);
        float v[4][4];
        bool ok[4];
#pragma unroll
        for (int k = 0; k < 4; ++k) {
            const int h = 2 * ho + (k >> 1), w = 2 * wo + (k & 1);
            ok[k] = h < H && w < W;
            float4 t = f4(-INFINITY);
            if (ok[k]) t = ld4(x + ((((size_t)n * H + h) * W + w) * C4 + c) * 4);
            v[k][0] = t.x; v[k][1] = t.y; v[k][2] = t.z; v[k][3] = t.w;
        }
        const float gv[4] = {g.x, g.y, g.z, g.w};
        float o[4][4];
#pragma unroll
        for (int e = 0; e < 4; ++e) {
            int arg = 0;
            float best = v[0][e];
#pragma unroll
            for (int k = 1; k < 4; ++k)
                if (v[k][e] > best) { best = v[k][e]; arg = k; }
#pragma unroll
            for (int k = 0; k < 4; ++k) o[k][e] = (k == arg) ? gv[e] : 0.f;
        }
#pragma unroll
        for (int k = 0; k < 4; ++k) {
            const int h = 2 * ho + (k >> 1), w = 2 * wo + (k & 1);
            if (ok[k]) st4(gx + ((((size_t)n * H + h) * W + w) * C4 + c) * 4, make_float4(o[k][0], o[k][1], o[k][2], o[k][3]));
        }
    }
}

__global__ __launch_bounds__(NT) void k_upsample_add(const float *__restrict__ top, const float *__restrict__ lat,
                                                     float *__restrict__ out, int N, int H, int W, int Ht, int Wt, int C4) {
    const size_t n4 = (size_t)N * H * W * C4;
    for (size_t i = (size_t)blockIdx.x * NT + threadIdx.x; i < n4; i += (size_t)gridDim.x * NT) {
        const Nhwc4 ix = split_nhwc4(i, C4, W, H, n4 > 0xFFFFFFFFull);
        const int c = ix.c, w = ix.w, h = ix.h, n = ix.n;
        const float4 a = ld4(top + ((((size_t)n * Ht + (h >> 1)) * Wt + (w >> 1)) * C4 + c) * 4);
        const float4 b = ld4(lat + i * 4);
        st4(out + i * 4, make_float4(a.x + b.x, a.y + b.y, a.z + b.z, a.w + b.w));
    }
}

__global__ __launch_bounds__(NT) void k_upsample_bwd(const float *__restrict__ gout, float *__restrict__ gtop, int N,
                                                     int H, int W, int Ht, int Wt, int C4, int accumulate) {
    const size_t n4 = (size_t)N * Ht * Wt * C4;
    for (size_t i = (size_t)blockIdx.x * NT + threadIdx.x; i < n4; i += (size_t)gridDim.x * NT) {
        const Nhwc4 ix = split_nhwc4(i, C4, Wt, Ht, n4 > 0xFFFFFFFFull);
        const int c = ix.c, wt = ix.w, ht = ix.h, n = ix.n;
        float4 s = accumulate ? ld4(gtop + i * 4) : f4(0.f);
#pragma unroll
        for (int dy = 0; dy < 2; ++dy)
#pragma unroll
            for (int dx = 0; dx < 2; ++dx) {
                const int h = 2 * ht + dy, w = 2 * wt + dx;
                if (h < H && w < W) {
                    const float4 v = ld4(gout + ((((size_t)n * H + h) * W + w) * C4 + c) * 4);
                    s.x += v.x; s.y += v.y; s.z += v.z; s.w += v.w;
                }
            }
        st4(gtop + i * 4, s);
    }
}

__global__ __launch_bounds__(NT) void k_subsample_bwd(const float *__restrict__ gsub, float *__restrict__ gx, int N,
                                                      int H, int W, int Ho, int Wo, int C4, int s, int accumulate,
                                                      const float *__restrict__ relu_x) {
    const size_t n4 = (size_t)N * H * W * C4;
    for (size_t i = (size_t)blockIdx.x * NT + threadIdx.x; i < n4; i += (size_t)gridDim.x * NT) {
        const Nhwc4 ix = split_nhwc4(i, C4, W, H, n4 > 0xFFFFFFFFull);
        const int c = ix.c, w = ix.w, h = ix.h, n = ix.n;
        const bool on = (h % s == 0) && (w % s == 0) && (h / s < Ho) && (w / s < Wo);
        if (accumulate) {
            if (!on) continue;
            const float4 g = ld4(gsub + ((((size_t)n * Ho + h / s) * Wo + w / s) * C4 + c) * 4);
            const float4 o = ld4(gx + i * 4);
            float4 v = make_float4(o.x + g.x, o.y + g.y, o.z + g.z, o.w + g.w);
            if (relu_x) {
                const float4 xm = ld4(relu_x + i * 4);
                v.x = xm.x > 0.f ? v.x : 0.f; v.y = xm.y > 0.f ? v.y : 0.f; v.z = xm.z > 0.f ? v.z : 0.f; v.w = xm.w > 0.f ? v.w : 0.f;
            }
            st4(gx + i * 4, v);
        } else {
            float4 g = f4(0.f);
            if (on) {
                g = ld4(gsub + ((((size_t)n * Ho + h / s) * Wo + w / s) * C4 + c) * 4);
                if (relu_x) {
                    const float4 xm = ld4(relu_x + i * 4);
                    g.x = xm.x > 0.f ? g.x : 0.f; g.y = xm.y > 0.f ? g.y : 0.f; g.z = xm.z > 0.f ? g.z : 0.f; g.w = xm.w > 0.f ? g.w : 0.f;
                }
            }
            st4(gx + i * 4, g);
        }
    }
}

__global__ __launch_bounds__(NT) void k_pixel_shuffle(const float *__restrict__ src, const float *__restrict__ bias,
                                                      float *__restrict__ dst, int N, int H, int W, int C4, int dir) {
    const size_t n4 = (size_t)N * H * W * 4 * C4;
    for (size_t i = (size_t)blockIdx.x * NT + threadIdx.x; i < n4; i += (size_t)gridDim.x * NT) {
        const Nhwc4 ix = split_nhwc4(i, C4, 2 * W, 2 * H, n4 > 0xFFFFFFFFull);
        const int c = ix.c, w2 = ix.w, h2 = ix.h, n = ix.n;
        const size_t j = ((((size_t)n * H + (h2 >> 1)) * W + (w2 >> 1)) * 4 + (h2 & 1) * 2 + (w2 & 1)) * C4 + c;
        if (dir == 0) {
            float4 v = ld4(src + j * 4);
            if (bias) { const float4 b = ld4(bias + c * 4); v.x += b.x; v.y += b.y; v.z += b.z; v.w += b.w; }
            st4(dst + i * 4, v);
        } else st4(dst + j * 4, ld4(src + i * 4));
    }
}

// ... 234 lines not shown

extern "C" size_t mrcnn_bn_workspace_bytes(int P, int C) {
    if (P <= 0 || C <= 0 || (C % 4)) return 0;
    const RedPlan r = red_plan(P, C);
    return (size_t)r.nblk * 2 * C * sizeof(float);
}

int g_bn_debug_skip = 0;
extern "C" int mrcnn_debug_bn_skip(int mask) {
    if (mask < 0 || mask > 3) return mrcnn::fail_arg(MRCNN_E_INVALID, "debug_bn_skip: mask in [0,3]");
    g_bn_debug_skip = mask;
    return 0;
}

extern "C" int mrcnn_debug_bn_plan(int red_cap, int fin_quads) {
    if (red_cap < 1 || red_cap > 8192 || (fin_quads != 1 && fin_quads != 4)) return mrcnn::fail_arg(MRCNN_E_INVALID, "debug_bn_plan: red_cap 1..8192, fin_quads 1 or 4");
    g_red_cap = red_cap; g_fin_quads = fin_quads;
    return 0;
}

extern "C" int mrcnn_bn_train_fwd_f32(const float *x, const float *gamma, const float *beta, const float *residual,
                                      float *y, float *save_mean, float *save_invstd, float *running_mean,
                                      float *running_var, int P, int C, float eps, float decay, int relu, void *ws,
                                      size_t ws_bytes, void *stream) {
    if (int e = chk(x && gamma && beta && y && save_mean && save_invstd && ws, "bn_train_fwd: null pointer")) return e;
    if (int e = chk(P > 0 && C > 0 && (C % 4) == 0, "bn_train_fwd: need P>0, C%4==0")) return e;
    if (ws_bytes < mrcnn_bn_workspace_bytes(P, C)) return mrcnn::fail_arg(MRCNN_E_WORKSPACE, "bn_train_fwd: workspace too small");
    hipStream_t st = (hipStream_t)stream;
    if (int e = launch_bn_stats(st, x, nullptr, 0, P, C, eps, decay, ws, save_mean, save_invstd, running_mean, running_var)) return e;
    const size_t n4 = (size_t)P * C / 4;
    hipLaunchKernelGGL(k_bn_apply, dim3(ew_grid(n4)), dim3(NT), 0, st, x, gamma, beta, save_mean, save_invstd, residual, y,
                       n4, C / 4, relu);
    MRCNN_LAUNCH_CHECK();
    return 0;
}

extern "C" int mrcnn_bn_train_fwd_stats_f32(const float *x, const float *part, int rows, const float *gamma, const float *beta,
                                            const float *residual, float *y, float *save_mean, float *save_invstd,
                                            float *running_mean, float *running_var, int P, int C, float eps, float decay, int relu,
                                            void *stream) {
    if (int e = chk(x && part && gamma && beta && y && save_mean && save_invstd, "bn_train_fwd_stats: null pointer")) return e;
    if (int e = chk(P > 0 && C > 0 && (C % 4) == 0 && rows > 0, "bn_train_fwd_stats: need P>0, C%4==0, rows>0")) return e;
    hipStream_t st = (hipStream_t)stream;
    if (!(g_bn_debug_skip & 2))
        if (int e = launch_bn_stats(st, x, part, rows, P, C, eps, decay, nullptr, save_mean, save_invstd, running_mean, running_var)) return e;
    const size_t n4 = (size_t)P * C / 4;
    hipLaunchKernelGGL(k_bn_apply, dim3(ew_grid(n4)), dim3(NT), 0, st, x, gamma, beta, save_mean, save_invstd, residual, y, n4, C / 4, relu);
    MRCNN_LAUNCH_CHECK();
    return 0;
}

extern "C" int mrcnn_bn_train_bwd_f32(const float *gy, const float *x, const float *y, const float *gamma, const float *beta,
                                      const float *save_mean, const float *save_invstd, float *gx, float *gres,
                                      float *ggamma, float *gbeta, int P, int C, int relu, void *ws, size_t ws_bytes,
                                      void *stream) {
    if (int e = chk(gy && x && gamma && save_mean && save_invstd && gx && ggamma && gbeta && ws, "bn_train_bwd: null pointer")) return e;
    if (int e = chk(!relu || y || beta, "bn_train_bwd: relu needs y, or beta to recompute the mask")) return e;
    const int rmode = !relu ? 0 : (y ? 1 : 2);
    if (int e = chk(P > 0 && C > 0 && (C % 4) == 0, "bn_train_bwd: need P>0, C%4==0")) return e;
    if (ws_bytes < mrcnn_bn_workspace_bytes(P, C)) return mrcnn::fail_arg(MRCNN_E_WORKSPACE, "bn_train_bwd: workspace too small");
    hipStream_t st = (hipStream_t)stream;
    const RedPlan r = red_plan(P, C);
    hipLaunchKernelGGL(k_bn_bwd_partial, dim3(r.nblk), dim3(NT), 0, st, gy, x, y, gamma, beta, save_mean, save_invstd, P, C, r.G,
                       r.RPI, r.rows_per_blk, rmode, (float *)ws);
    MRCNN_LAUNCH_CHECK();
    if (!(g_bn_debug_skip & 1))
    launch_bwd_final(st, (const float *)ws, r.nblk, C, gbeta, ggamma);
    MRCNN_LAUNCH_CHECK();
    const size_t n4 = (size_t)P * C / 4;
    hipLaunchKernelGGL(k_bn_bwd_apply, dim3(ew_grid(n4)), dim3(NT), 0, st, gy, x, y, gamma, save_mean, save_invstd, gbeta,
                       ggamma, gx, gres, n4, C / 4, 1.0f / (float)P, rmode, beta);
    MRCNN_LAUNCH_CHECK();
    return 0;
}

extern "C" int mrcnn_bn_train_stats_f32(const float *x, const float *part, int rows, float *save_mean, float *save_invstd, float *running_mean,
                                        float *running_var, int P, int C, float eps, float decay, void *ws, size_t ws_bytes, void *stream) {
    if (int e = chk(x && save_mean && save_invstd, "bn_train_stats: null pointer")) return e;
    if (int e = chk(P > 0 && C > 0 && (C % 4) == 0 && rows >= 0 && (rows == 0) == (part == nullptr), "bn_train_stats: need P>0, C%4==0, part / rows together")) return e;
    if (!part && (!ws || ws_bytes < mrcnn_bn_workspace_bytes(P, C))) return mrcnn::fail_arg(MRCNN_E_WORKSPACE, "bn_train_stats: workspace too small");
    return launch_bn_stats((hipStream_t)stream, x, part, rows, P, C, eps, decay, ws, save_mean, save_invstd, running_mean, running_var);
}

extern "C" size_t mrcnn_bn_pair_workspace_bytes(int P, int C) {
    if (P <= 0 || C <= 0 || (C % 4)) return 0;
    const RedPlan r = red_plan(P, C);
    return (size_t)r.nblk * 3 * C * sizeof(float);
}

extern "C" int mrcnn_bn_train_fwd_pair_f32(const float *xa, const float *part_a, int rows_a, const float *gamma_a, const float *beta_a,
                                           float *mean_a, float *invstd_a, float *run_mean_a, float *run_var_a, const float *xb,
                                           const float *part_b, int rows_b, const float *gamma_b, const float *beta_b, float *mean_b,
                                           float *invstd_b, float *run_mean_b, float *run_var_b, float *y, int P, int C, float eps, float decay,
                                           void *ws, size_t ws_bytes, void *stream) {
    if (int e = chk(xa && gamma_a && beta_a && mean_a && invstd_a && xb && gamma_b && beta_b && mean_b && invstd_b && y, "bn_train_fwd_pair: null pointer")) return e;
    if (int e = chk(P > 0 && C > 0 && (C % 4) == 0 && rows_a >= 0 && rows_b >= 0, "bn_train_fwd_pair: need P>0, C%4==0, rows>=0")) return e;
    if (int e = chk((rows_a == 0) == (part_a == nullptr) && (rows_b == 0) == (part_b == nullptr), "bn_train_fwd_pair: part / rows must come together")) return e;
    if ((!part_a || !part_b) && (!ws || ws_bytes < mrcnn_bn_workspace_bytes(P, C)))
        return mrcnn::fail_arg(MRCNN_E_WORKSPACE, "bn_train_fwd_pair: a statistics pass needs mrcnn_bn_workspace_bytes() of workspace");
    hipStream_t st = (hipStream_t)stream;
    if (int e = launch_bn_stats(st, xb, part_b, rows_b, P, C, eps, decay, ws, mean_b, invstd_b, run_mean_b, run_var_b)) return e;
    if (int e = launch_bn_stats(st, xa, part_a, rows_a, P, C, eps, decay, ws, mean_a, invstd_a, run_mean_a, run_var_a)) return e;
    const size_t n4 = (size_t)P * C / 4;
    hipLaunchKernelGGL(k_bn_apply2, dim3(ew_grid(n4)), dim3(NT), 0, st, xa, gamma_a, beta_a, mean_a, invstd_a, xb, gamma_b, beta_b, mean_b, invstd_b, y,
                       n4, C / 4);
    MRCNN_LAUNCH_CHECK();
    return 0;
}

extern "C" int mrcnn_bn_train_bwd_pair_f32(const float *gy, const float *y, const float *xa, const float *xb, const float *gamma_a,
                                           const float *mean_a, const float *invstd_a, const float *gamma_b, const float *mean_b,
                                           const float *invstd_b, float *gxa, float *gxb, float *ggamma_a, float *gbeta_a, float *ggamma_b,
                                           float *gbeta_b, int P, int C, void *ws, size_t ws_bytes, void *stream) {
    if (int e = chk(gy && xa && xb && gamma_a && mean_a && invstd_a && gamma_b && mean_b && invstd_b && gxa && gxb && ggamma_a && gbeta_a && ggamma_b &&
                        gbeta_b && ws, "bn_train_bwd_pair: null pointer")) return e;
    if (int e = chk(P > 0 && C > 0 && (C % 4) == 0, "bn_train_bwd_pair: need P>0, C%4==0")) return e;
    if (ws_bytes < mrcnn_bn_pair_workspace_bytes(P, C)) return mrcnn::fail_arg(MRCNN_E_WORKSPACE, "bn_train_bwd_pair: workspace too small");
    hipStream_t st = (hipStream_t)stream;
    const RedPlan r = red_plan(P, C);
    hipLaunchKernelGGL(k_bn_bwd_partial2, dim3(r.nblk), dim3(NT), 0, st, gy, y, xa, xb, mean_a, invstd_a, mean_b, invstd_b, P, C, r.G, r.RPI,
                       r.rows_per_blk, (float *)ws);
    MRCNN_LAUNCH_CHECK();
    launch_bwd_final2(st, (const float *)ws, r.nblk, C, gbeta_a, ggamma_a, gbeta_b, ggamma_b);
    MRCNN_LAUNCH_CHECK();
    const size_t n4 = (size_t)P * C / 4;
    hipLaunchKernelGGL(k_bn_bwd_apply2, dim3(ew_grid(n4)), dim3(NT), 0, st, gy, y, xa, xb, gamma_a, mean_a, invstd_a, gbeta_a, ggamma_a, gamma_b, mean_b,
                       invstd_b, gbeta_b, ggamma_b, gxa, gxb, n4, C / 4, 1.0f / (float)P);
    MRCNN_LAUNCH_CHECK();
    return 0;
}

extern "C" int mrcnn_relu_bwd_f32(const float *gy, const float *y, float *gx, size_t n, void *stream) {
    if (n == 0) return 0;
    if (int e = chk(gy && y && gx && (n % 4) == 0, "relu_bwd: null pointer or n%4")) return e;
    hipLaunchKernelGGL(k_relu_bwd, dim3(ew_grid(n / 4)), dim3(NT), 0, (hipStream_t)stream, gy, y, gx, n / 4);
    MRCNN_LAUNCH_CHECK();
    return 0;
}

extern "C" int mrcnn_add_f32(const float *a, const float *b, float *out, size_t n, void *stream) {
    if (n == 0) return 0;
    if (int e = chk(a && b && out && (n % 4) == 0, "add: null pointer or n%4")) return e;
    hipLaunchKernelGGL(k_add, dim3(ew_grid(n / 4)), dim3(NT), 0, (hipStream_t)stream, a, b, out, n / 4);
    MRCNN_LAUNCH_CHECK();
    return 0;
}

extern "C" int mrcnn_maxpool2x2_fwd_f32(const float *x, float *y, int N, int H, int W, int C, void *stream) {
    if (int e = chk(x && y && N > 0 && H > 0 && W > 0 && C > 0 && (C % 4) == 0, "maxpool2x2_fwd: bad args")) return e;
    const int Ho = (H + 1) / 2, Wo = (W + 1) / 2;
    hipLaunchKernelGGL(k_maxpool_fwd, dim3(ew_grid((size_t)N * Ho * Wo * C / 4)), dim3(NT), 0, (hipStream_t)stream, x, y,
                       N, H, W, C / 4, Ho, Wo);
    MRCNN_LAUNCH_CHECK();
    return 0;
}

extern "C" int mrcnn_maxpool3x3s2_fwd_f32(const float *x, float *y, int N, int H, int W, int C, void *stream) {
    if (int e = chk(x && y && N > 0 && H >= 3 && W >= 3 && C > 0 && (C % 4) == 0, "maxpool3x3s2_fwd: bad args")) return e;
    const int Ho = (H - 3 + 1) / 2 + 1, Wo = (W - 3 + 1) / 2 + 1;
    hipLaunchKernelGGL(k_maxpool3s2_fwd, dim3(ew_grid((size_t)N * Ho * Wo * C / 4)), dim3(NT), 0, (hipStream_t)stream, x, y, N, H, W,
                       C / 4, Ho, Wo);
    MRCNN_LAUNCH_CHECK();
    return 0;
}

extern "C" int mrcnn_global_avg_pool_fwd_f32(const float *x, float *y, int R, int P, int C, void *stream) {
// ... 194 lines not shown
```

include/mrcnn_hip.h:

```cpp
#ifndef MRCNN_HIP_H
#define MRCNN_HIP_H

#include <stddef.h>
#include <stdint.h>

#ifdef __cplusplus
extern "C" {
#endif

#define MRCNN_ABI_VERSION 10

enum {
    MRCNN_OK = 0,
    MRCNN_E_INVALID = -1,
    MRCNN_E_UNSUPPORTED = -2,
    MRCNN_E_WORKSPACE = -3
};

enum { MRCNN_LAYOUT_NCHW = 0, MRCNN_LAYOUT_NHWC = 1 };

#define MRCNN_MAX_LEVELS 8

int mrcnn_abi_version(void);
const char *mrcnn_last_error(void);
// ... 32 lines not shown
size_t mrcnn_roi_align_fpn_bwd_plan_bytes(const int *Hs, const int *Ws, int L, int N, int R, int PH, int PW, int split_levels);
int mrcnn_roi_align_fpn_bwd_plan_f32(const int *Hs, const int *Ws, const float *scales, int L, int N, int C, const float *rois,
                                     const int32_t *levels, int R, int PH, int PW, int sampling_ratio, int split_levels,
                                     void *plan, size_t plan_bytes, void *stream);
int mrcnn_debug_roi_align_lean_variant(int v);
int mrcnn_debug_roi_align_lean_stamps(unsigned long long *stamps);
int mrcnn_roi_align_fpn_bwd_planned_f32(const float *gy, float *const *gxs, const int *Hs, const int *Ws, const float *scales, int L,
                                        int N, int C, const float *rois, const int32_t *levels, int R, int PH, int PW,
                                        int sampling_ratio, int accumulate, void *ws, size_t ws_bytes, void *plan,
                                        size_t plan_bytes, int plan_verified, void *stream);
int mrcnn_roi_align_bwd_plan_status(const void *plan, size_t plan_bytes, int *status3, void *stream);

int mrcnn_roi_align_set_bwd_variant(int variant);

int mrcnn_debug_roi_align_bwd_stamps(const float *gy, int N, int C, int H, int W, const float *rois, int R, int PH, int PW,
                                     float spatial_scale, int sampling_ratio, float *gx, unsigned long long *stamps,
                                     void *stream);

int mrcnn_debug_dispatch_census(unsigned long long *out, int nblocks, int spin_us, void *stream);

int mrcnn_roi_align_sample_tables(const float *rois, int R, int H, int W, int PH, int PW,
                                  float spatial_scale, int sampling_ratio, int smax,
                                  int32_t *cnt, int32_t *idx, float *wgt, void *stream);

size_t mrcnn_conv2d_workspace_bytes(int N, int H, int W, int Cin, int Cout, int KH, int KW, int stride, int pad);
long long mrcnn_conv2d_executed_macs(int N, int H, int W, int Cin, int Cout, int KH, int KW, int stride, int pad, int pass);
int mrcnn_conv2d_set_winograd_thresholds(int min_channels, int min_pixels, int tile);
int mrcnn_conv2d_set_winograd_pass_tiles(int fwd, int bwd_data, int bwd_filter);
int mrcnn_conv2d_get_winograd_pass_tiles(int *tiles3);
int mrcnn_conv2d_set_split_operands(int fwd, int bwd_data, int bwd_filter);
int mrcnn_conv2d_get_split_operands(int *modes3);
#define MRCNN_CONV_PLAN_FIELDS 9
int mrcnn_conv2d_plan_query(int pass, int N, int H, int W, int Cin, int Cout, int KH, int KW, int stride, int pad, int *out, int n_out);
int mrcnn_debug_conv_plan(int fill, int filter_rounds, int force_tile);
int mrcnn_debug_wino_banded(int on);
int mrcnn_debug_conv_parts(int mask);
int mrcnn_debug_split_planes_f32(const float *x, void *planes, int R, int C, int r4, void *stream);
int mrcnn_debug_planes_gemm_stamps(unsigned long long *stamps);
int mrcnn_debug_planes_gemm(int kind, const void *a, const void *b, float *c, int M, int N, int K, int batch_rows, int nbatch,
                            int ksplit, int bm, int bn, void *stream);

int mrcnn_conv2d_set_debug_skip(int mask);
int mrcnn_debug_bn_skip(int mask);
int mrcnn_debug_bn_plan(int red_cap, int fin_quads);
size_t mrcnn_conv2d_winograd_v_bytes(int N, int H, int W, int Cin, int Cout, int KH, int KW, int stride, int pad);
int mrcnn_conv2d_fwd_f32(const float *x, const float *w, const float *bias, float *y, int N, int H,
                         int W, int Cin, int Cout, int KH, int KW, int stride, int pad, int relu,
                         float *wino_v, void *ws, size_t ws_bytes, void *stream);
size_t mrcnn_conv2d_bnstats_rows(int N, int H, int W, int Cin, int Cout, int KH, int KW, int stride, int pad);
int mrcnn_conv2d_fwd_bnstats_f32(const float *x, const float *w, float *y, int N, int H, int W, int Cin, int Cout, int KH, int KW,
                                 int stride, int pad, float *bn_part, float *wino_v, void *ws, size_t ws_bytes, void *stream);
int mrcnn_conv2d_fwd_rect_f32(const float *x, const float *w, const float *bias, float *y, int N, int H, int W, int Cin,
                              int Cout, int KH, int KW, int stride, int pad_h, int pad_w, int relu, void *ws,
                              size_t ws_bytes, void *stream);
size_t mrcnn_conv2d_winograd_w_bytes(int N, int H, int W, int Cin, int Cout, int KH, int KW, int stride, int pad);
int mrcnn_conv2d_bwd_data_f32(const float *gy, const float *w, float *gx, const float *relu_x, int N, int H, int W, int Cin,
                              int Cout, int KH, int KW, int stride, int pad, int accumulate, float *wino_w,
                              float *gbias, int gbias_accumulate, void *ws, size_t ws_bytes, void *stream);
size_t mrcnn_conv2d_bwd_filter_workspace_bytes(int N, int H, int W, int Cin, int Cout, int KH, int KW,
                                               int stride, int pad);
int mrcnn_conv2d_bwd_filter_f32(const float *x, const float *gy, float *gw, float *gbias, int N, int H,
                                int W, int Cin, int Cout, int KH, int KW, int stride, int pad, int accumulate,
                                const float *wino_v, const float *wino_w,
                                void *ws, size_t ws_bytes, void *stream);

size_t mrcnn_bn_workspace_bytes(int P, int C);
int mrcnn_bn_train_fwd_f32(const float *x, const float *gamma, const float *beta, const float *residual,
                           float *y, float *save_mean, float *save_invstd, float *running_mean,
                           float *running_var, int P, int C, float eps, float decay, int relu, void *ws,
                           size_t ws_bytes, void *stream);
int mrcnn_bn_train_fwd_stats_f32(const float *x, const float *part, int rows, const float *gamma, const float *beta,
                                 const float *residual, float *y, float *save_mean, float *save_invstd, float *running_mean,
                                 float *running_var, int P, int C, float eps, float decay, int relu, void *stream);
int mrcnn_bn_train_bwd_f32(const float *gy, const float *x, const float *y, const float *gamma, const float *beta,
                           const float *save_mean, const float *save_invstd, float *gx, float *gres,
                           float *ggamma, float *gbeta, int P, int C, int relu, void *ws, size_t ws_bytes,
                           void *stream);
int mrcnn_bn_train_stats_f32(const float *x, const float *part, int rows, float *save_mean, float *save_invstd, float *running_mean,
                             float *running_var, int P, int C, float eps, float decay, void *ws, size_t ws_bytes, void *stream);
int mrcnn_conv2d_inbn_ok(int N, int H, int W, int Cin, int Cout, int KH, int KW, int stride, int pad);
int mrcnn_conv2d_fwd_inbn_f32(const float *x, const float *in_gamma, const float *in_beta, const float *in_mean, const float *in_invstd,
                              const float *w, float *y, int N, int H, int W, int Cin, int Cout, int KH, int KW, int stride, int pad,
                              float *bn_part, float *wino_v, void *ws, size_t ws_bytes, void *stream);
int mrcnn_conv2d_bwd_filter_inbn_f32(const float *x, const float *in_gamma, const float *in_beta, const float *in_mean,
                                     const float *in_invstd, const float *gy, float *gw, int N, int H, int W, int Cin, int Cout, int KH,
                                     int KW, int stride, int pad, int accumulate, const float *wino_v, void *ws, size_t ws_bytes,
                                     void *stream);
size_t mrcnn_bn_pair_workspace_bytes(int P, int C);
int mrcnn_bn_train_fwd_pair_f32(const float *xa, const float *part_a, int rows_a, const float *gamma_a, const float *beta_a,
                                float *mean_a, float *invstd_a, float *run_mean_a, float *run_var_a, const float *xb,
                                const float *part_b, int rows_b, const float *gamma_b, const float *beta_b, float *mean_b,
                                float *invstd_b, float *run_mean_b, float *run_var_b, float *y, int P, int C, float eps, float decay,
                                void *ws, size_t ws_bytes, void *stream);
int mrcnn_bn_train_bwd_pair_f32(const float *gy, const float *y, const float *xa, const float *xb, const float *gamma_a,
                                const float *mean_a, const float *invstd_a, const float *gamma_b, const float *mean_b,
                                const float *invstd_b, float *gxa, float *gxb, float *ggamma_a, float *gbeta_a, float *ggamma_b,
                                float *gbeta_b, int P, int C, void *ws, size_t ws_bytes, void *stream);
int mrcnn_bn_infer_fwd_f32(const float *x, const float *gamma, const float *beta, const float *mean,
                           const float *var, const float *residual, float *y, int P, int C, float eps, int relu,
                           void *stream);
int mrcnn_relu_bwd_f32(const float *gy, const float *y, float *gx, size_t n, void *stream);
int mrcnn_add_f32(const float *a, const float *b, float *out, size_t n, void *stream);
int mrcnn_maxpool2x2_fwd_f32(const float *x, float *y, int N, int H, int W, int C, void *stream);
int mrcnn_maxpool2x2_bwd_f32(const float *x, const float *gy, float *gx, int N, int H, int W, int C, void *stream);
int mrcnn_maxpool3x3s2_fwd_f32(const float *x, float *y, int N, int H, int W, int C, void *stream);
int mrcnn_global_avg_pool_fwd_f32(const float *x, float *y, int R, int P, int C, void *stream);
int mrcnn_relu_fwd_f32(const float *x, float *y, size_t n, void *stream);
int mrcnn_upsample2x_add_fwd_f32(const float *top, const float *lat, float *out, int N, int H, int W, int Ht,
                                 int Wt, int C, void *stream);
int mrcnn_upsample2x_bwd_f32(const float *gout, float *gtop, int N, int H, int W, int Ht, int Wt, int C,
                             int accumulate, void *stream);
int mrcnn_subsample_bwd_f32(const float *gsub, float *gx, int N, int H, int W, int C, int stride, int accumulate,
                            const float *relu_x, void *stream);
int mrcnn_pixel_shuffle2x_f32(const float *src, const float *bias, float *dst, int N, int H, int W, int C, int inverse,
                              void *stream);
int mrcnn_deconv_merge_fwd_f32(const float *wd, const float *bd, const float *w2, const float *b2, float *wm,
                               float *bm, int C, int Cin, int K2, int ld2, void *stream);
int mrcnn_deconv_merge_bwd_f32(const float *G, const float *gb4, const float *wd, const float *bd,
                               const float *w2, float *gwd, float *gbd, float *gw2, float *gb2, int C,
                               int Cin, int K2, int ld2, void *stream);
int mrcnn_bilinear2x_fwd_f32(const float *x, float *y, int N, int H, int W, int C, void *stream);
int mrcnn_bilinear2x_bwd_f32(const float *gy, float *gx, int N, int H, int W, int C, void *stream);
int mrcnn_image_nchw3_to_nhwc4_f32(const float *x, float *y, int N, int H, int W, void *stream);
int mrcnn_image_resize_u8_f32(const uint8_t *src, int H, int W, float *dst, int oh, int ow, int dst_h, int dst_w,
                              float div, void *stream);
int mrcnn_mask_resize_nearest_u8(const uint8_t *src, int G, int H, int W, uint8_t *dst, int oh, int ow, int dst_h,
                                 int dst_w, void *stream);
int mrcnn_image_resize_f32(const float *src, int C, int H, int W, float *dst, int oh, int ow, int dst_h, int dst_w,
                           float div, void *stream);
int mrcnn_random_keys_u32(uint32_t *out, size_t n, unsigned long long seed, void *stream);
int mrcnn_random_keys_dev_u32(uint32_t *out, size_t n, unsigned long long *state, void *stream);
int mrcnn_sgd_momentum_wd_f32(float *p, const float *g, float *v, size_t n, float lr, float momentum,
                              float weight_decay, void *stream);

typedef struct mrcnn_bottleneck {
    int32_t N, H, W;
    int32_t cin, mid, cout;
    int32_t stride, project;
    int32_t fwd_split;
    float eps, decay;
    const float *w[4];
    const float *gamma[4];
    const float *beta[4];
    float *run_mean[4];
    float *run_var[4];
    float *gw[4];
    float *ggamma[4];
    float *gbeta[4];
} mrcnn_bottleneck_t;

enum { MRCNN_BN_H1 = 0, MRCNN_BN_A1, MRCNN_BN_H2, MRCNN_BN_A2, MRCNN_BN_H3, MRCNN_BN_H4, MRCNN_BN_R,
       MRCNN_BN_V = 7 , MRCNN_BN_PART = 11 , MRCNN_BN_MEAN = 15 , MRCNN_BN_INVSTD = 19 ,
       MRCNN_BN_SLOTS = 23 };

typedef struct mrcnn_bottleneck_plan {
    uint64_t arena_bytes;
    uint64_t ws_bytes;
    uint64_t off[MRCNN_BN_SLOTS];
    uint64_t v_bytes[4];
    int32_t part_rows[4];
} mrcnn_bottleneck_plan_t;

int mrcnn_debug_bottleneck_inbn(int on);
int mrcnn_bottleneck_fwd_plan(const mrcnn_bottleneck_t *b, mrcnn_bottleneck_plan_t *plan);
int mrcnn_bottleneck_fwd_f32(const mrcnn_bottleneck_t *b, const mrcnn_bottleneck_plan_t *plan, const float *x, float *y,
                             void *arena, size_t arena_bytes, void *ws, size_t ws_bytes, void *stream);
int mrcnn_bottleneck_bwd_sizes(const mrcnn_bottleneck_t *b, size_t *sizes3);
int mrcnn_bottleneck_bwd_f32(const mrcnn_bottleneck_t *b, const mrcnn_bottleneck_plan_t *plan, const float *x, const float *y,
                             const void *fwd_arena, const float *gy, int gy_masked, float *g_r, float *gx_acc, float *gx_new,
                             int mask_gx, void *arena, size_t arena_bytes, void *ws_main, size_t ws_main_bytes, void *ws_side,
                             size_t ws_side_bytes, void *stream, void *side_stream);

size_t mrcnn_loss_workspace_bytes(void);
int mrcnn_softmax_ce_fills_gx(int M, int K, int A, long long gs, long long rs, long long es, long long ggs, long long grs, long long ges,
                              int Kfill);
int mrcnn_softmax_ce_f32(const float *x, int A, long long gs, long long rs, long long es, const int32_t *t,
                         int M, int K, int ignore_label, float *loss_out, float *gx, long long ggs,
                         long long grs, long long ges, int Kfill, void *ws, size_t ws_bytes, void *stream);
int mrcnn_smooth_l1_f32(const float *x, int ldx, const float *t, const int32_t *label, int M, float sigma,
                        float *loss_out, float *gx, int ldg, int gfill, void *ws, size_t ws_bytes, void *stream);
// ... 199 lines not shown
```

Before: 96.50.

## Fuse stem BN+ReLU+maxpool and FPN upsample-add into Winograd input transform

Adds fused kernels that apply stem BatchNorm, ReLU and the 2x2 maxpool in one pass, with a matching backward that recomputes the BN output and pool argmax from x. The FPN top-down upsample-add is folded into the Winograd input transform of the following 3x3 conv, which reads the coarser top map at half resolution. The aim is to avoid materialising the stem BN output and the summed FPN merge tensors, cutting HBM traffic and kernel launches. The cost is extra recompute in the backward pass. The Winograd V tensor is cached from the fused input, so the backward filter pass must use the same tile size, which the new eligibility check enforces.

```diff
diff --git a/__graft_entry__.py b/__graft_entry__.py
--- a/__graft_entry__.py
+++ b/__graft_entry__.py
@@ -15,6 +15,7 @@
     oc = os.path.join(ROOT, 'oracle', 'c')
     if os.path.exists(os.path.join(oc, 'Makefile')):
         subprocess.check_call(['make', '-C', oc])
+    import torch
     from chainer_maskrcnn import _hip
     _hip._lib = None
     assert _hip.lib().mrcnn_abi_version() == _hip.ABI_VERSION
diff --git a/chainer-maskrcnn_amd/chainer_maskrcnn/_hip/nn.py b/chainer-maskrcnn_amd/chainer_maskrcnn/_hip/nn.py
--- a/chainer-maskrcnn_amd/chainer_maskrcnn/_hip/nn.py
+++ b/chainer-maskrcnn_amd/chainer_maskrcnn/_hip/nn.py
@@ -135,6 +135,25 @@
     return y, v, part
 
 
+def conv2d_fwd_inadd_raw(lat, top, w, b, keep_v=True):
+    _hip.require_cuda(lat, top, w)
+    N, H, W, Cin = lat.shape
+    Cout, KH, KW, Cin2 = w.shape
+    assert Cin == Cin2 == top.shape[3] and top.shape[0] == N, (lat.shape, top.shape, w.shape)
+    if not lib().mrcnn_conv2d_inadd_ok(N, H, W, Cin, Cout, KH, KW, 1, 1):
+        return None
+    assert lat.is_contiguous() and top.is_contiguous() and w.is_contiguous()
+    y = torch.empty((N, H, W, Cout), dtype=torch.float32, device=lat.device)
+    ws = workspace(lib().mrcnn_conv2d_workspace_bytes(N, H, W, Cin, Cout, KH, KW, 1, 1), lat.device)
+    v = None
+    if keep_v:
+        v = torch.empty((lib().mrcnn_conv2d_winograd_v_bytes(N, H, W, Cin, Cout, KH, KW, 1, 1) // 4,), dtype=torch.float32, device=lat.device)
+    with _prof('fwd', N * H * W, KH, KW, Cin, Cout, (N, H, W, Cin, Cout, KH, KW, 1, 1)):
+        check(lib().mrcnn_conv2d_fwd_inadd_f32(ptr(lat), ptr(top), top.shape[1], top.shape[2], ptr(w), ptr(b), ptr(y), N, H, W, Cin, Cout, KH, KW,
+                                               1, 1, ptr(v), ptr(ws), ws.numel(), stream_ptr()))
+    return y, v
+
+
 def winograd_w_bytes(x_shape, w_shape, stride, pad):
     N, H, W, Cin = x_shape
     Cout, KH, KW, _ = w_shape
diff --git a/chainer-maskrcnn_amd/chainer_maskrcnn/_hip/ops.py b/chainer-maskrcnn_amd/chainer_maskrcnn/_hip/ops.py
--- a/chainer-maskrcnn_amd/chainer_maskrcnn/_hip/ops.py
+++ b/chainer-maskrcnn_amd/chainer_maskrcnn/_hip/ops.py
@@ -62,6 +62,32 @@
     check(lib().mrcnn_bn_train_bwd_f32(ptr(gy), ptr(x), ptr(y), ptr(gamma), ptr(beta), ptr(mean), ptr(invstd), ptr(gx), ptr(gres),
                                        ptr(gg), ptr(gb), P, C, int(relu), ptr(ws), ws.numel(), stream_ptr()))
     return gx, gres, gg, gb
+
+
+def bn_relu_maxpool2x2_fwd(x, gamma, beta, running_mean=None, running_var=None, eps=2e-5, decay=0.9):
+    _ck(x, gamma, beta)
+    N, H, W, C = x.shape
+    y = _empty((N, H // 2, W // 2, C), x.device)
+    mean = _empty((C,), x.device)
+    invstd = _empty((C,), x.device)
+    ws = workspace(lib().mrcnn_bn_workspace_bytes(N * H * W, C), x.device)
+    check(lib().mrcnn_bn_relu_maxpool2x2_fwd_f32(ptr(x), ptr(gamma), ptr(beta), ptr(y), ptr(mean), ptr(invstd), ptr(running_mean),
+                                                 ptr(running_var), N, H, W, C, eps, decay, ptr(ws), ws.numel(), stream_ptr()))
+    return y, mean, invstd
+
+
+def bn_relu_maxpool2x2_bwd(gy, x, gamma, beta, mean, invstd, gg=None, gb=None):
+    _ck(gy, x, gamma, beta, mean, invstd, gg, gb)
+    N, H, W, C = x.shape
+    if tuple(gy.shape) != (N, H // 2, W // 2, C):
+        raise ValueError('bn_relu_maxpool2x2_bwd: gy %r does not match x %r' % (tuple(gy.shape), tuple(x.shape)))
+    gx = torch.empty_like(x)
+    gg = _empty((C,), x.device) if gg is None else gg
+    gb = _empty((C,), x.device) if gb is None else gb
+    ws = workspace(lib().mrcnn_bn_workspace_bytes(N * H * W, C), x.device)
+    check(lib().mrcnn_bn_relu_maxpool2x2_bwd_f32(ptr(gy), ptr(x), ptr(gamma), ptr(beta), ptr(mean), ptr(invstd), ptr(gx), ptr(gg), ptr(gb),
+                                                 N, H, W, C, ptr(ws), ws.numel(), stream_ptr()))
+    return gx, gg, gb
 
 
 def bn_infer_fwd(x, gamma, beta, mean, var, residual=None, relu=False, eps=2e-5):
diff --git a/chainer-maskrcnn_amd/chainer_maskrcnn/model/extractor/feature_pyramid_network.py b/chainer-maskrcnn_amd/chainer_maskrcnn/model/extractor/feature_pyramid_network.py
--- a/chainer-maskrcnn_amd/chainer_maskrcnn/model/extractor/feature_pyramid_network.py
+++ b/chainer-maskrcnn_amd/chainer_maskrcnn/model/extractor/feature_pyramid_network.py
@@ -4,6 +4,8 @@
 MASK_IN_PRODUCER = True
 LATERALS_OFF_THE_CHAIN = False
 _lat_streams = {}
+FUSE_STEM_POOL = True
+FUSE_TOPDOWN_ADD = True
 
 
 def _lateral_stream(device):
@@ -83,12 +85,15 @@
         t = {}
         stem_trained = self.freeze_at < 1
         h, t['conv1'] = self.conv1.fwd(x, tape=stem_trained)
-        h, t['bn1'] = self.bn1.fwd(h, relu=True)
-        if stem_trained:
-            t['pool_in'] = h
+        if FUSE_STEM_POOL and stem_trained and self.bn1.pool_fusable(h):
+            h, t['bn1_pool'] = self.bn1.fwd_relu_pool(h)
         else:
-            t['bn1'] = None
-        h = ops.maxpool2x2_fwd(h)
+            h, t['bn1'] = self.bn1.fwd(h, relu=True)
+            if stem_trained:
+                t['pool_in'] = h
+            else:
+                t['bn1'] = None
+            h = ops.maxpool2x2_fwd(h)
         cs = []
         t['blocks'] = []
         off_chain = LATERALS_OFF_THE_CHAIN and x.is_cuda and hnn.PROFILE is None
@@ -113,14 +118,11 @@
                 l_.record_stream(main)
         p5, t['top'] = self.toplayer.fwd(c5)
         l4, t['lat4'] = lat[2] if off_chain else self.lat_p4.fwd(c4)
-        m4 = ops.upsample2x_add_fwd(p5, l4)
-        p4, t['p4'] = self.conv_p4.fwd(m4)
+        p4, t['p4'] = self.conv_p4.fwd_topdown(p5, l4, fuse=FUSE_TOPDOWN_ADD)
         l3, t['lat3'] = lat[1] if off_chain else self.lat_p3.fwd(c3)
-        m3 = ops.upsample2x_add_fwd(p4, l3)
-        p3, t['p3'] = self.conv_p3.fwd(m3)
+        p3, t['p3'] = self.conv_p3.fwd_topdown(p4, l3, fuse=FUSE_TOPDOWN_ADD)
         l2, t['lat2'] = lat[0] if off_chain else self.lat_p2.fwd(c2)
-        m2 = ops.upsample2x_add_fwd(p3, l2)
-        p2, t['p2'] = self.conv_p2.fwd(m2)
+        p2, t['p2'] = self.conv_p2.fwd_topdown(p3, l2, fuse=FUSE_TOPDOWN_ADD)
         p6, t['p6'] = self.conv_p6.fwd(p5)
         self.tape = t
         return p2, p3, p4, p5, p6
@@ -179,7 +181,10 @@
                         progress(b.conv1.name)
             self.tape = None
             return
-        g = ops.maxpool2x2_bwd(t['pool_in'], g)
-        g, _ = self.bn1.bwd(t['bn1'], g)
+        if 'bn1_pool' in t:
+            g = self.bn1.bwd_relu_pool(t['bn1_pool'], g)
+        else:
+            g = ops.maxpool2x2_bwd(t['pool_in'], g)
+            g, _ = self.bn1.bwd(t['bn1'], g)
         self.conv1.bwd(t['conv1'], g, need_gx=False)
         self.tape = None
diff --git a/chainer-maskrcnn_amd/chainer_maskrcnn/nn/core.py b/chainer-maskrcnn_amd/chainer_maskrcnn/nn/core.py
--- a/chainer-maskrcnn_amd/chainer_maskrcnn/nn/core.py
+++ b/chainer-maskrcnn_amd/chainer_maskrcnn/nn/core.py
@@ -195,6 +195,17 @@
                 (hnn.conv2d_fwd_raw(x, self.W, self.b, self.stride, self.pad, relu), None)
         hnn.LOGICAL = None
         return y, (x, y if relu else None, v)
+
+    def fwd_topdown(self, top, lat, fuse=True):
+        if fuse and TRAIN and not self.relu and self.k == 3 and self.stride == 1 and self.pad == 1:
+            hnn.LOGICAL = (self.cin, self.cout)
+            with _layer_tiles(self):
+                res = hnn.conv2d_fwd_inadd_raw(lat, top, self.W, self.b)
+            hnn.LOGICAL = None
+            if res is not None:
+                self.last_bn_part = None
+                return res[0], (lat, None, res[1])
+        return self.fwd(ops.upsample2x_add_fwd(top, lat))
 
     def bwd(self, ctx, gy, need_gx=True, gx_acc=None, accumulate_params=False, gy_masked=False, mask_gx=False):
         with _layer_tiles(self):
@@ -284,6 +295,21 @@
                                                self.ps.buffers[self.name + '/avg_var'])
         return y, (x, y if (residual is not None or not relu) else None, mean, invstd, relu)
 
+    def pool_fusable(self, x):
+        return TRAIN and not self.frozen and x.shape[1] % 2 == 0 and x.shape[2] % 2 == 0
+
+    def fwd_relu_pool(self, x):
+        gamma, beta = self.ps.p(self.name + '/gamma'), self.ps.p(self.name + '/beta')
+        y, mean, invstd = ops.bn_relu_maxpool2x2_fwd(x, gamma, beta, self.ps.buffers[self.name + '/avg_mean'],
+                                                     self.ps.buffers[self.name + '/avg_var'])
+        return y, (x, mean, invstd)
+
+    def bwd_relu_pool(self, ctx, gy):
+        x, mean, invstd = ctx
+        gx, _, _ = ops.bn_relu_maxpool2x2_bwd(gy, x, self.ps.p(self.name + '/gamma'), self.ps.p(self.name + '/beta'), mean, invstd,
+                                              gg=self.ps.g(self.name + '/gamma'), gb=self.ps.g(self.name + '/beta'))
+        return gx
+
     def scale_operands(self):
         return self.ps.p(self.name + '/gamma'), self.ps.buffers[self.name + '/avg_var']
 
diff --git a/chainer-maskrcnn_amd/csrc/conv.hip b/chainer-maskrcnn_amd/csrc/conv.hip
--- a/chainer-maskrcnn_amd/csrc/conv.hip
+++ b/chainer-maskrcnn_amd/csrc/conv.hip
@@ -1284,10 +1284,11 @@
     __builtin_amdgcn_raw_buffer_store_b128(d, rs, voff, soff, 0);
 }
 struct InBN { const float *gamma, *beta, *mean, *invstd; };
-template <int M_>
+struct InAdd { const float *top; int Ht, Wt; };
+template <int M_, bool ADD = false>
 __device__ __forceinline__ void wino_input_body(const float *__restrict__ x, float *__restrict__ V, int N, int H, int W, int C,
                                                 int th, int tw, long long T, long long Tp, unsigned blk, const InBN bn = InBN{},
-                                                int panel = 0) {
+                                                int panel = 0, const InAdd add = InAdd{}) {
     constexpr int A_ = M_ + 2;
     const unsigned C4 = (unsigned)C / 4u;
     const unsigned i = blk * 256u + threadIdx.x;
@@ -1329,6 +1330,16 @@
         rowo[r] = (unsigned)h < (unsigned)H ? (unsigned)(((size_t)n * H + h) * W * C * 4) : OOB;
         colo[r] = (unsigned)ww < (unsigned)W ? (unsigned)(((size_t)ww * C + c) * 4) : OOB;
     }
+    const auto rsT = __builtin_amdgcn_make_buffer_rsrc((void *)(ADD ? add.top : x), 0, ADD ? (unsigned)((size_t)N * add.Ht * add.Wt * C * 4) : 0u, 0x00020000);
+    unsigned rowt[A_], colt[A_];
+    if (ADD) {
+#pragma unroll
+        for (int r = 0; r < A_; ++r) {
+            const int h = M_ * ty - 1 + r, ww = M_ * tx - 1 + r;
+            rowt[r] = (unsigned)h < (unsigned)H ? (unsigned)(((size_t)n * add.Ht + (h >> 1)) * add.Wt * C * 4) : OOB;
+            colt[r] = (unsigned)ww < (unsigned)W ? (unsigned)(((size_t)(ww >> 1) * C + c) * 4) : OOB;
+        }
+    }
     V4 bg = v4zero(), bb = v4zero(), bm = v4zero(), bs = v4zero();
     if (bn.gamma) { bg = v4ld(bn.gamma + c); bb = v4ld(bn.beta + c); bm = v4ld(bn.mean + c); bs = v4ld(bn.invstd + c); }
     V4 b[A_][A_];
@@ -1337,6 +1348,13 @@
         V4 d[A_], r[A_];
 #pragma unroll
         for (int rr = 0; rr < A_; ++rr) d[rr] = v4buf(rsX, (rowo[rr] == OOB || colo[q] == OOB) ? OOB : rowo[rr] + colo[q], 0);
+        if (ADD) {
+            V4 e[A_];
+#pragma unroll
+            for (int rr = 0; rr < A_; ++rr) e[rr] = v4buf(rsT, (rowt[rr] == OOB || colt[q] == OOB) ? OOB : rowt[rr] + colt[q], 0);
+#pragma unroll
+            for (int rr = 0; rr < A_; ++rr) d[rr] = e[rr] + d[rr];
+        }
         if (bn.gamma) {
 #pragma unroll
             for (int rr = 0; rr < A_; ++rr) {
@@ -1380,6 +1398,15 @@
                                                            int banded, int uplanes, InBN bn) {
     if (blockIdx.x < fblocks) wino_filter_body<M_>(w, U, Cout_w, Cin_w, transposed, blockIdx.x, uplanes);
     else wino_input_body<M_>(x, V, N, H, W, C, th, tw, T, Tp, xcd_banded(blockIdx.x, fblocks, gridDim.x - fblocks, banded), bn, banded);
+}
+
+template <int M_>
+__global__ __launch_bounds__(256) void k_wino_input_filter_add(const float *__restrict__ x, float *__restrict__ V, int N, int H, int W, int C,
+                                                               int th, int tw, long long T, long long Tp, const float *__restrict__ w,
+                                                               float *__restrict__ U, int Cout_w, int Cin_w, unsigned fblocks, int banded,
+                                                               int uplanes, InAdd add) {
+    if (blockIdx.x < fblocks) wino_filter_body<M_>(w, U, Cout_w, Cin_w, 0, blockIdx.x, uplanes);
+    else wino_input_body<M_, true>(x, V, N, H, W, C, th, tw, T, Tp, xcd_banded(blockIdx.x, fblocks, gridDim.x - fblocks, banded), InBN{}, banded, add);
 }
 
 template <int M_>
@@ -1718,6 +1745,7 @@
 }
 
 thread_local InBN t_inbn{};
+thread_local InAdd t_inadd{};
 
 int wino_bwd_filter(const float *x, const float *gy, float *gw, int N, int H, int W, int Cin, int Cout, int accumulate, void *ws,
                     hipStream_t st, const float *v_cached, const float *w_cached, float *bias_part = nullptr, int *bias_rows = nullptr) {
@@ -1812,7 +1840,10 @@
             if (!(g_debug_skip & 2)) hipLaunchKernelGGL(k_colsum_final, dim3(mrcnn::cdiv(Cin, CSF_CH)), dim3(CSF_CH * CSF_SL), 0, st, part, gbias, cp.nblk, Cin, gbias_accumulate);
             MRCNN_LAUNCH_CHECK();
         }
-    } else
+    } else if (!transposed && t_inadd.top)
+        WINO_LAUNCH(k_wino_input_filter_add, g, dim3(fblocks + (unsigned)((nin + 255) / 256)), in, V, N, H, W, Cin, g.th, g.tw, g.T, g.Tp, w, U,
+                    Cout, Cin, fblocks, g_wino_banded, big, t_inadd);
+    else
         WINO_LAUNCH(k_wino_input_filter, g, dim3(fblocks + (unsigned)((nin + 255) / 256)), in, V, N, H, W, Cin, g.th, g.tw, g.T, g.Tp, w, U,
                     transposed ? Cin : Cout, transposed ? Cout : Cin, transposed ? 1 : 0, fblocks, g_wino_banded, big, inbn);
     if (big) {
@@ -2151,6 +2182,26 @@
     return rc;
 }
 
+extern "C" int mrcnn_conv2d_inadd_ok(int N, int H, int W, int Cin, int Cout, int KH, int KW, int stride, int pad) {
+    if (!mrcnn_conv2d_inbn_ok(N, H, W, Cin, Cout, KH, KW, stride, pad)) return 0;
+    return wino_geom(N, H, W, PASS_FWD).m == wino_geom(N, H, W, PASS_BWD_FILTER).m ? 1 : 0;
+}
+extern "C" int mrcnn_conv2d_fwd_inadd_f32(const float *lat, const float *top, int Ht, int Wt, const float *w, const float *bias, float *y, int N,
+                                          int H, int W, int Cin, int Cout, int KH, int KW, int stride, int pad, float *wino_v, void *ws,
+                                          size_t ws_bytes, void *stream) {
+    if (!lat || !top || !w || !y) return mrcnn::fail_arg(MRCNN_E_INVALID, "conv2d_fwd_inadd: null pointer");
+    if (!mrcnn_conv2d_inadd_ok(N, H, W, Cin, Cout, KH, KW, stride, pad))
+        return mrcnn::fail_arg(MRCNN_E_UNSUPPORTED, "conv2d_fwd_inadd: this geometry does not take the Winograd path on one tile in both passes (mrcnn_conv2d_inadd_ok == 0)");
+    if (Ht < (H + 1) / 2 || Wt < (W + 1) / 2) return mrcnn::fail_arg(MRCNN_E_INVALID, "conv2d_fwd_inadd: top smaller than ceil(out/2)");
+    if ((long long)N * Ht * Wt * Cin * 4 >= (1ll << 32)) return mrcnn::fail_arg(MRCNN_E_UNSUPPORTED, "conv2d_fwd_inadd: top of 4 GiB or more");
+    if (!ws || ws_bytes < wino_ws_bytes(N, H, W, Cin, Cout, PASS_FWD))
+        return mrcnn::fail_arg(MRCNN_E_WORKSPACE, "conv2d_fwd_inadd: workspace %zu < %zu", ws_bytes, wino_ws_bytes(N, H, W, Cin, Cout, PASS_FWD));
+    t_inadd = InAdd{top, Ht, Wt};
+    const int rc = mrcnn_conv2d_fwd_f32(lat, w, bias, y, N, H, W, Cin, Cout, KH, KW, stride, pad, 0, wino_v, ws, ws_bytes, stream);
+    t_inadd = InAdd{};
+    return rc;
+}
+
 extern "C" int mrcnn_conv2d_fwd_rect_f32(const float *x, const float *w, const float *bias, float *y, int N, int H, int W,
                                          int Cin, int Cout, int KH, int KW, int stride, int pad_h, int pad_w, int relu, void *ws,
                                          size_t ws_bytes, void *stream) {
diff --git a/chainer-maskrcnn_amd/csrc/nn.hip b/chainer-maskrcnn_amd/csrc/nn.hip
--- a/chainer-maskrcnn_amd/csrc/nn.hip
+++ b/chainer-maskrcnn_amd/csrc/nn.hip
@@ -501,6 +501,15 @@
     }
 }
 
+__device__ __forceinline__ int maxpool_arg1(float v0, float v1, float v2, float v3) {
+    int arg = 0;
+    float best = v0;
+    if (v1 > best) { best = v1; arg = 1; }
+    if (v2 > best) { best = v2; arg = 2; }
+    if (v3 > best) { best = v3; arg = 3; }
+    return arg;
+}
+
 __global__ __launch_bounds__(NT) void k_maxpool_bwd(const float *__restrict__ x, const float *__restrict__ gy,
                                                     float *__restrict__ gx, int N, int H, int W, int C4, int Ho, int Wo) {
     const size_t n4 = (size_t)N * Ho * Wo * C4;
@@ -522,11 +531,7 @@
         float o[4][4];
 #pragma unroll
         for (int e = 0; e < 4; ++e) {
-            int arg = 0;
-            float best = v[0][e];
-#pragma unroll
-            for (int k = 1; k < 4; ++k)
-                if (v[k][e] > best) { best = v[k][e]; arg = k; }
+            const int arg = maxpool_arg1(v[0][e], v[1][e], v[2][e], v[3][e]);
 #pragma unroll
             for (int k = 0; k < 4; ++k) o[k][e] = (k == arg) ? gv[e] : 0.f;
         }
@@ -535,6 +540,110 @@
             const int h = 2 * ho + (k >> 1), w = 2 * wo + (k & 1);
             if (ok[k]) st4(gx + ((((size_t)n * H + h) * W + w) * C4 + c) * 4, make_float4(o[k][0], o[k][1], o[k][2], o[k][3]));
         }
+    }
+}
+
+struct StemWin { float4 v[4], o[4]; };
+__device__ __forceinline__ StemWin stem_window(const float *__restrict__ x, size_t tl, int W, int C, const float4 &ga, const float4 &m,
+                                               const float4 &s, const float4 &be) {
+    StemWin w;
+    w.v[0] = ld4(x + tl); w.v[1] = ld4(x + tl + C); w.v[2] = ld4(x + tl + (size_t)W * C); w.v[3] = ld4(x + tl + (size_t)W * C + C);
+#pragma unroll
+    for (int k = 0; k < 4; ++k) w.o[k] = bn_affine4(w.v[k], ga, m, s, be);
+    return w;
+}
+__device__ __forceinline__ void stem_args(const StemWin &w, int (&arg)[4]) {
+    float4 a[4];
+#pragma unroll
+    for (int k = 0; k < 4; ++k) a[k] = relu4(w.o[k]);
+    arg[0] = maxpool_arg1(a[0].x, a[1].x, a[2].x, a[3].x); arg[1] = maxpool_arg1(a[0].y, a[1].y, a[2].y, a[3].y);
+    arg[2] = maxpool_arg1(a[0].z, a[1].z, a[2].z, a[3].z); arg[3] = maxpool_arg1(a[0].w, a[1].w, a[2].w, a[3].w);
+}
+__device__ __forceinline__ float4 stem_dz(const float4 &g, const int (&arg)[4], int k, const float4 &o) {
+    const float4 gp = make_float4(arg[0] == k ? g.x : 0.f, arg[1] == k ? g.y : 0.f, arg[2] == k ? g.z : 0.f, arg[3] == k ? g.w : 0.f);
+    return relu_mask4(gp, o);
+}
+
+__global__ __launch_bounds__(NT) void k_bn_relu_maxpool_fwd(const float *__restrict__ x, const float *__restrict__ gamma,
+                                                            const float *__restrict__ beta, const float *__restrict__ mean,
+                                                            const float *__restrict__ invstd, float *__restrict__ y, int N, int H, int W,
+                                                            int C4) {
+    const int Ho = H / 2, Wo = W / 2, C = C4 * 4;
+    const size_t n4 = (size_t)N * Ho * Wo * C4;
+    for (size_t i = (size_t)blockIdx.x * NT + threadIdx.x; i < n4; i += (size_t)gridDim.x * NT) {
+        const Nhwc4 ix = split_nhwc4(i, C4, Wo, Ho, n4 > 0xFFFFFFFFull);
+        const int c = ix.c * 4;
+        const float4 ga = ld4(gamma + c), be = ld4(beta + c), m = ld4(mean + c), s = ld4(invstd + c);
+        const StemWin w = stem_window(x, (((size_t)ix.n * H + 2 * ix.h) * W + 2 * ix.w) * C + c, W, C, ga, m, s, be);
+        float4 mx = f4(-INFINITY);
+#pragma unroll
+        for (int k = 0; k < 4; ++k) {
+            const float4 a = relu4(w.o[k]);
+            mx.x = fmaxf(mx.x, a.x); mx.y = fmaxf(mx.y, a.y); mx.z = fmaxf(mx.z, a.z); mx.w = fmaxf(mx.w, a.w);
+        }
+        st4(y + i * 4, mx);
+    }
+}
+
+__global__ __launch_bounds__(NT) void k_bn_relu_maxpool_bwd_partial(const float *__restrict__ gy, const float *__restrict__ x,
+                                                                    const float *__restrict__ gamma, const float *__restrict__ beta,
+                                                                    const float *__restrict__ mean, const float *__restrict__ invstd,
+                                                                    int P, int H, int W, int C, int G, int RPI, int rows_per_blk,
+                                                                    float *__restrict__ part) {
+    __shared__ float4 s1[NT], s2[NT];
+    const int t = threadIdx.x, cg0 = t % G, rr = t / G;
+    const int C4 = C / 4;
+    const int r0 = blockIdx.x * rows_per_blk, r1 = min(P, r0 + rows_per_blk);
+    const unsigned HW = (unsigned)H * (unsigned)W, Wo = (unsigned)W / 2u;
+    for (int cg = cg0; cg < C4; cg += G) {
+        const float4 m = ld4(mean + cg * 4), s = ld4(invstd + cg * 4), ga = ld4(gamma + cg * 4), be = ld4(beta + cg * 4);
+        float4 a = f4(0.f), b = f4(0.f);
+        for (int r = r0 + rr; r < r1; r += RPI) {
+            const unsigned n = (unsigned)r / HW, q = (unsigned)r - n * HW, h = q / (unsigned)W, w = q - h * (unsigned)W;
+            const int k = (int)((h & 1u) * 2u + (w & 1u));
+            const StemWin win = stem_window(x, ((size_t)r - (h & 1u) * (unsigned)W - (w & 1u)) * C + cg * 4, W, C, ga, m, s, be);
+            const float4 g = ld4(gy + ((size_t)(n * (HW / 4u) + (h >> 1) * Wo + (w >> 1))) * C + cg * 4);
+            int arg[4];
+            stem_args(win, arg);
+            float4 v = win.v[0], o = win.o[0];
+#pragma unroll
+            for (int j = 1; j < 4; ++j)
+                if (k == j) { v = win.v[j]; o = win.o[j]; }
+            bn_bwd_acc4(stem_dz(g, arg, k, o), v, m, s, a, b);
+        }
+        s1[t] = a; s2[t] = b;
+        __syncthreads();
+        if (rr == 0) {
+            for (int k = 1; k < RPI; ++k) {
+                const float4 p = s1[k * G + cg0], q = s2[k * G + cg0];
+                a = add4(a, p); b = add4(b, q);
+            }
+            st4(part + ((size_t)blockIdx.x * 2 * C) + cg * 4, a);
+            st4(part + ((size_t)blockIdx.x * 2 * C) + C + cg * 4, b);
+        }
+        __syncthreads();
+    }
+}
+
+__global__ __launch_bounds__(NT) void k_bn_relu_maxpool_bwd_apply(const float *__restrict__ gy, const float *__restrict__ x,
+                                                                  const float *__restrict__ gamma, const float *__restrict__ beta,
+                                                                  const float *__restrict__ mean, const float *__restrict__ invstd,
+                                                                  const float *__restrict__ gbeta, const float *__restrict__ ggamma,
+                                                                  float *__restrict__ gx, int N, int H, int W, int C4, float invP) {
+    const int Ho = H / 2, Wo = W / 2, C = C4 * 4;
+    const size_t n4 = (size_t)N * Ho * Wo * C4;
+    for (size_t i = (size_t)blockIdx.x * NT + threadIdx.x; i < n4; i += (size_t)gridDim.x * NT) {
+        const Nhwc4 ix = split_nhwc4(i, C4, Wo, Ho, n4 > 0xFFFFFFFFull);
+        const int c = ix.c * 4;
+        const float4 ga = ld4(gamma + c), be = ld4(beta + c), m = ld4(mean + c), s = ld4(invstd + c), gb = ld4(gbeta + c), gg = ld4(ggamma + c);
+        const size_t tl = (((size_t)ix.n * H + 2 * ix.h) * W + 2 * ix.w) * C + c;
+        const StemWin w = stem_window(x, tl, W, C, ga, m, s, be);
+        const float4 g = ld4(gy + i * 4);
+        int arg[4];
+        stem_args(w, arg);
+#pragma unroll
+        for (int k = 0; k < 4; ++k)
+            st4(gx + tl + (size_t)(k >> 1) * W * C + (size_t)(k & 1) * C, bn_bwd_dx4(stem_dz(g, arg, k, w.o[k]), w.v[k], ga, m, s, gb, gg, invP));
     }
 }
 
@@ -935,6 +1044,47 @@
     return launch_bn_stats((hipStream_t)stream, x, part, rows, P, C, eps, decay, ws, save_mean, save_invstd, running_mean, running_var);
 }
 
+static int stem_args_ok(bool ptrs, int N, int H, int W, int C, void *ws, size_t ws_bytes, const char *who) {
+    if (!ptrs || !ws) return mrcnn::fail_arg(MRCNN_E_INVALID, "%s: null pointer", who);
+    if (N <= 0 || H <= 0 || W <= 0 || C <= 0 || (C % 4) || (long long)N * H * W > 0x7FFFFFFFll)
+        return mrcnn::fail_arg(MRCNN_E_INVALID, "%s: need N, H, W > 0, C %% 4 == 0, N*H*W < 2^31", who);
+    if ((H % 2) || (W % 2)) return mrcnn::fail_arg(MRCNN_E_UNSUPPORTED, "%s: odd H or W (%d x %d): run the BatchNorm and the pool separately", who, H, W);
+    if (ws_bytes < mrcnn_bn_workspace_bytes(N * H * W, C)) return mrcnn::fail_arg(MRCNN_E_WORKSPACE, "%s: workspace too small", who);
+    return 0;
+}
+extern "C" int mrcnn_bn_relu_maxpool2x2_fwd_f32(const float *x, const float *gamma, const float *beta, float *y, float *save_mean,
+                                                float *save_invstd, float *running_mean, float *running_var, int N, int H, int W, int C,
+                                                float eps, float decay, void *ws, size_t ws_bytes, void *stream) {
+    if (int e = stem_args_ok(x && gamma && beta && y && save_mean && save_invstd, N, H, W, C, ws, ws_bytes, "bn_relu_maxpool2x2_fwd")) return e;
+    hipStream_t st = (hipStream_t)stream;
+    const int P = N * H * W;
+    if (int e = launch_bn_stats(st, x, nullptr, 0, P, C, eps, decay, ws, save_mean, save_invstd, running_mean, running_var)) return e;
+    hipLaunchKernelGGL(k_bn_relu_maxpool_fwd, dim3(ew_grid((size_t)P / 4 * (C / 4))), dim3(NT), 0, st, x, gamma, beta, save_mean, save_invstd, y,
+                       N, H, W, C / 4);
+    MRCNN_LAUNCH_CHECK();
+    return 0;
+}
+
+extern "C" int mrcnn_bn_relu_maxpool2x2_bwd_f32(const float *gy, const float *x, const float *gamma, const float *beta, const float *save_mean,
+                                                const float *save_invstd, float *gx, float *ggamma, float *gbeta, int N, int H, int W, int C,
+                                                void *ws, size_t ws_bytes, void *stream) {
+    if (int e = stem_args_ok(gy && x && gamma && beta && save_mean && save_invstd && gx && ggamma && gbeta, N, H, W, C, ws, ws_bytes,
+                             "bn_relu_maxpool2x2_bwd")) return e;
+    hipStream_t st = (hipStream_t)stream;
+    const int P = N * H * W;
+    const RedPlan r = red_plan(P, C);
+    hipLaunchKernelGGL(k_bn_relu_maxpool_bwd_partial, dim3(r.nblk), dim3(NT), 0, st, gy, x, gamma, beta, save_mean, save_invstd, P, H, W, C, r.G,
+                       r.RPI, r.rows_per_blk, (float *)ws);
+    MRCNN_LAUNCH_CHECK();
+    if (!(g_bn_debug_skip & 1))
+    launch_bwd_final(st, (const float *)ws, r.nblk, C, gbeta, ggamma);
+    MRCNN_LAUNCH_CHECK();
+    hipLaunchKernelGGL(k_bn_relu_maxpool_bwd_apply, dim3(ew_grid((size_t)P / 4 * (C / 4))), dim3(NT), 0, st, gy, x, gamma, beta, save_mean,
+                       save_invstd, gbeta, ggamma, gx, N, H, W, C / 4, 1.0f / (float)P);
+    MRCNN_LAUNCH_CHECK();
+    return 0;
+}
+
 extern "C" size_t mrcnn_bn_pair_workspace_bytes(int P, int C) {
     if (P <= 0 || C <= 0 || (C % 4)) return 0;
     const RedPlan r = red_plan(P, C);
diff --git a/include/mrcnn_hip.h b/include/mrcnn_hip.h
--- a/include/mrcnn_hip.h
+++ b/include/mrcnn_hip.h
@@ -138,6 +138,10 @@
 int mrcnn_conv2d_fwd_inbn_f32(const float *x, const float *in_gamma, const float *in_beta, const float *in_mean, const float *in_invstd,
                               const float *w, float *y, int N, int H, int W, int Cin, int Cout, int KH, int KW, int stride, int pad,
                               float *bn_part, float *wino_v, void *ws, size_t ws_bytes, void *stream);
+int mrcnn_conv2d_inadd_ok(int N, int H, int W, int Cin, int Cout, int KH, int KW, int stride, int pad);
+int mrcnn_conv2d_fwd_inadd_f32(const float *lat, const float *top, int Ht, int Wt, const float *w, const float *bias, float *y, int N,
+                               int H, int W, int Cin, int Cout, int KH, int KW, int stride, int pad, float *wino_v, void *ws,
+                               size_t ws_bytes, void *stream);
 int mrcnn_conv2d_bwd_filter_inbn_f32(const float *x, const float *in_gamma, const float *in_beta, const float *in_mean,
                                      const float *in_invstd, const float *gy, float *gw, int N, int H, int W, int Cin, int Cout, int KH,
                                      int KW, int stride, int pad, int accumulate, const float *wino_v, void *ws, size_t ws_bytes,
@@ -152,6 +156,12 @@
                                 const float *mean_a, const float *invstd_a, const float *gamma_b, const float *mean_b,
                                 const float *invstd_b, float *gxa, float *gxb, float *ggamma_a, float *gbeta_a, float *ggamma_b,
                                 float *gbeta_b, int P, int C, void *ws, size_t ws_bytes, void *stream);
+int mrcnn_bn_relu_maxpool2x2_fwd_f32(const float *x, const float *gamma, const float *beta, float *y, float *save_mean,
+                                     float *save_invstd, float *running_mean, float *running_var, int N, int H, int W, int C,
+                                     float eps, float decay, void *ws, size_t ws_bytes, void *stream);
+int mrcnn_bn_relu_maxpool2x2_bwd_f32(const float *gy, const float *x, const float *gamma, const float *beta, const float *save_mean,
+                                     const float *save_invstd, float *gx, float *ggamma, float *gbeta, int N, int H, int W, int C,
+                                     void *ws, size_t ws_bytes, void *stream);
 int mrcnn_bn_infer_fwd_f32(const float *x, const float *gamma, const float *beta, const float *mean,
                            const float *var, const float *residual, float *y, int P, int C, float eps, int relu,
                            void *stream);
```

Result: no change. 96.23 (-0.3%).
